# adobe-research/DiffusionHandles

Hardware: AMD Instinct MI355X
Metric: guided-denoise steps/sec at 512x512 (SD2-depth) (higher is better)
Workload: dtype f16; 1 GPU; single 512x512 edit per GPU, SD2-depth (865.9M params, seeded random weights), guided phase: 3 x (fwd + energy + bwd-to-latent) + CFG fwd (B=2) + DDIM step; resolution=512, edits_per_gpu=1, correspondences=24906, parallelism=independent edits, one process per GPU, no collectives

## Files before the change

diffusionhandles_amd/_lib.py:

```python
import ctypes
import os

import torch

_HERE = os.path.dirname(os.path.abspath(__file__))
LIB_PATH = os.environ.get("DIFFHANDLES_LIB") or os.path.join(_HERE, "libdiffhandles_hip.so")
_LIB = None

c_p = ctypes.c_void_p
c_i = ctypes.c_int
c_f = ctypes.c_float
c_d = ctypes.c_double
c_sz = ctypes.c_size_t


class UNetConfig(ctypes.Structure):
    _fields_ = [("in_channels", c_i), ("out_channels", c_i), ("n_levels", c_i),
                ("block_out_channels", c_i * 4), ("layers_per_block", c_i), ("heads", c_i * 4),
                ("cross_attention_dim", c_i), ("norm_groups", c_i), ("sample_size", c_i),
                ("text_len", c_i), ("max_batch", c_i), ("dtype", c_i), ("max_diff_batch", c_i)]


class VAEConfig(ctypes.Structure):
    _fields_ = [("latent_channels", c_i), ("out_channels", c_i), ("block_out_channels", c_i * 4),
# ... 70 lines not shown
    "dh_text_encoder_bytes": (c_sz, [c_p]),
    "dh_text_encoder_encode": (c_i, [c_p, c_p, c_i, c_i, c_p, c_p]),
    "dh_gemm_profile_begin": (c_i, []),
    "dh_gemm_profile_end": (c_i, [ctypes.POINTER(c_d), ctypes.POINTER(ctypes.c_int64), ctypes.POINTER(c_d)]),
    "dh_gemm_profile_bytes": (c_i, [ctypes.POINTER(c_d)]),
    "dh_ddim_cfg_step": (c_i, [c_p, c_p, c_p, c_p, c_f, c_f, c_f, c_i, c_p]),
    "dh_latent_update": (c_i, [c_p, c_p, c_p, c_f, c_f, c_i, c_p]),
    "dh_adam_step": (c_i, [c_p, c_p, c_p, c_p, c_f, c_f, c_f, c_f, c_i, c_i, c_p]),
    "dh_mse_fwd_bwd": (c_i, [c_p, c_p, c_i, c_p, c_p, c_p]),
    "dh_latent_update_strided": (c_i, [c_p, c_p, c_p, c_i, c_i, c_f, c_f, c_i, c_p]),
    "dh_pack_sample": (c_i, [c_p, c_p, c_i, c_i, c_p, c_i, c_i, c_i, c_i, c_p]),
    "dh_unet_io_ptr": (c_i, [c_p, c_i, c_i, ctypes.POINTER(c_p), ctypes.POINTER(c_sz)]),
    "dh_mse_cotangent": (c_i, [c_p, c_p, c_i, c_f, c_f, c_p, c_p, c_p, c_p]),
    "dh_adam_step_scaled": (c_i, [c_p, c_p, c_p, c_p, c_p, c_f, c_f, c_f, c_f, c_i, c_i, c_p]),
    "dh_mse_cotangent_batch": (c_i, [c_p, c_p, c_i, c_i, c_f, c_f, c_d, c_p, c_p, c_p, c_p, c_p, c_p]),
    "dh_adam_step_scaled_batch": (c_i, [c_p, c_p, c_p, c_p, c_p, c_p, c_f, c_f, c_f, c_f, c_i, c_i, c_i, c_p]),
    "dh_latent_update_guarded": (c_i, [c_p, c_p, c_p, c_i, c_i, c_f, c_i, c_i, c_p, c_i, c_i, c_p, c_p, c_i, c_i, c_p]),
    "dh_ddim_cfg_step_flagged": (c_i, [c_p, c_p, c_p, c_p, c_f, c_f, c_f, c_i, c_i, c_p, c_i, c_i, c_p]),
}

c_l = ctypes.c_long
DEBUG_SIGNATURES = {
    "dh_dbg_gemm": (c_i, [c_i, c_p, c_l, c_p, c_i, c_i, c_i, c_i, c_i, c_i, c_i, c_i, c_i, c_i, c_i, c_p, c_p, c_i, c_i,
                          c_p, c_l, c_p, c_l, c_i, c_p, c_sz, c_p]),
    "dh_dbg_gemm_groupnorm": (c_i, [c_i, c_p, c_l, c_p, c_i, c_i, c_i, c_i, c_i, c_i, c_i, c_p, c_p, c_p, c_sz, c_i, c_i, c_p, c_p, c_f, c_i,
                                    c_p, c_p, c_p, ctypes.POINTER(c_i), c_p]),
    "dh_dbg_gemm_groupnorm_bwd": (c_i, [c_i, c_p, c_l, c_p, c_i, c_i, c_i, c_i, c_i, c_i, c_i, c_p, c_p, c_sz, c_i, c_i, c_p, c_p, c_p, c_p, c_i,
                                        c_p, c_p, ctypes.POINTER(c_i), c_p]),
    "dh_dbg_gemm_groupnorm_res": (c_i, [c_i, c_p, c_l, c_p, c_i, c_i, c_i, c_i, c_i, c_i, c_i, c_p, c_p, c_l, c_p, c_p, c_sz, c_i, c_i, c_p, c_p,
                                    c_f, c_i, c_p, c_p, c_p, ctypes.POINTER(c_i), c_p]),
    "dh_dbg_gemm_groupnorm_bwd_res": (c_i, [c_i, c_p, c_l, c_p, c_i, c_i, c_i, c_i, c_i, c_i, c_i, c_p, c_l, c_p, c_p, c_sz, c_i, c_i, c_p, c_p, c_p,
                                        c_p, c_i, c_p, c_p, ctypes.POINTER(c_i), c_p]),
    "dh_dbg_concat_groupnorm": (c_i, [c_i, c_p, c_i, c_p, c_i, c_p, c_i, c_i, c_i, c_p, c_p, c_f, c_i, c_p, c_p, c_p, c_p]),
    "dh_dbg_gemm_last_tile": (c_i, [ctypes.POINTER(c_i)]),
    "dh_dbg_unet_concat_ops": (c_i, [ctypes.POINTER(UNetConfig), ctypes.POINTER(c_i), c_i, ctypes.POINTER(c_i)]),
    "dh_dbg_gemm_lnfold": (c_i, [c_i, c_p, c_l, c_p, c_i, c_i, c_i, c_p, c_p, c_p, c_f, c_p, c_l, c_p]),
    "dh_dbg_gemm_glu": (c_i, [c_i, c_i, c_p, c_l, c_p, c_i, c_i, c_i, c_p, c_p, c_p, c_p, c_p, c_p]),
    "dh_dbg_gemm_glub_split": (c_i, [c_i, c_p, c_l, c_p, c_i, c_i, c_i, c_i, c_p, c_l, c_i, c_p, c_p, ctypes.POINTER(c_i), c_p]),
    "dh_dbg_unet_ff_fold": (c_i, [c_p, c_i, ctypes.POINTER(c_i), ctypes.POINTER(c_i), c_p, c_p, c_p]),
    "dh_dbg_gemm_family": (c_i, [c_i]),
    "dh_dbg_gemm_stage": (c_i, [c_i]),
    "dh_dbg_gemm_pp_variant": (c_i, [c_i, c_p]),
    "dh_dbg_gemm_pp_ablate": (c_i, [c_i]),
    "dh_dbg_gemm_pp_persist": (c_i, [c_i]),
    "dh_dbg_gemm_pp_glu": (c_i, [c_i]),
    "dh_dbg_gemm_pp_plan": (c_i, [c_i, c_i, c_i, c_i, c_i, c_i, c_sz, ctypes.POINTER(c_i), ctypes.POINTER(c_i), ctypes.POINTER(c_i)]),
    "dh_dbg_touch_tiled": (c_i, [c_sz, c_p]),
    "dh_dbg_groupnorm": (c_i, [c_i, c_p, c_p, c_p, c_p, c_p, c_p, c_p, c_p, c_i, c_i, c_i, c_i, c_f, c_i, c_i, c_p]),
    "dh_dbg_layernorm": (c_i, [c_i, c_p, c_p, c_p, c_p, c_p, c_p, c_p, c_p, c_i, c_i, c_f, c_p]),
    "dh_dbg_geglu": (c_i, [c_i, c_p, c_p, c_p, c_p, c_i, c_i, c_p]),
    "dh_dbg_attention": (c_i, [c_i, c_p, c_l, c_p, c_p, c_l, c_p, c_l, c_p, c_p, c_p, c_p, c_p, c_p, c_i, c_i, c_i, c_i, c_p]),
    "dh_dbg_attention_bwd_pair": (c_i, [c_i, c_p, c_l, c_p, c_p, c_l, c_p, c_l, c_p, c_p, c_p, c_p, c_p, c_p, c_i, c_i, c_i, c_i, c_p, c_p]),
    "dh_dbg_pool2x2": (c_i, [c_i, c_p, c_p, c_i, c_i, c_i, c_i, c_i, c_p]),
    "dh_dbg_ellipse_offsets": (c_i, [c_i, ctypes.POINTER(ctypes.c_int32), c_i, ctypes.POINTER(c_i)]),
    "dh_dbg_lane_ops": (c_i, [c_p, c_p, c_p, c_p]),
}


def lib():
    global _LIB
    if _LIB is None:
        if not os.path.exists(LIB_PATH):
            raise RuntimeError(
                f"native HIP library not found at {LIB_PATH}; build it with "
                "`python -c 'import __graft_entry__ as g; g.build()'` (there is no CPU fallback)")
        handle = ctypes.CDLL(LIB_PATH)
        missing = []
# ... 40 lines not shown
```

diffusionhandles_amd/csrc/debug_api.cpp:

```cpp
#include <stdlib.h>

#include "unet_kernels.h"
using namespace dh;

static void* g_dbg_tiled = nullptr;

__global__ void k_dbg_touch(const uint4* p, size_t n16, unsigned* sink) {
  unsigned acc = 0;
  for (size_t i = (size_t)blockIdx.x * blockDim.x + threadIdx.x; i < n16; i += (size_t)gridDim.x * blockDim.x) { const uint4 v = p[i]; acc ^= v.x ^ v.y ^ v.z ^ v.w; }
  if (acc == 0x9e3779b9u && sink) sink[0] = acc;
}
extern "C" int dh_dbg_touch_tiled(size_t bytes, void* stream) {
  DH_REQUIRE(g_dbg_tiled != nullptr, "no tiled weights yet (call dh_dbg_gemm first)");
  hipLaunchKernelGGL(k_dbg_touch, dim3(512), dim3(256), 0, (hipStream_t)stream, (const uint4*)g_dbg_tiled, bytes / 16, (unsigned*)nullptr);
  DH_LAUNCH_CHECK();
  return DH_OK;
}

extern "C" int dh_dbg_gemm(int dtype, const void* A, long lda, const void* W, int M, int N, int K, int mode, int Hin,
                           int Win, int Cin, int Hout, int Wout, int stride, int up, const float* bias,
                           const float* rowvec, int rowvec_ld, int rows_per_batch, const void* R, long ldr, void* C,
                           long ldc, int act_silu, float* partial, size_t partial_elems, void* stream) {
  DH_REQUIRE(A && W && C && K % 64 == 0 && N % 64 == 0, "bad arguments (N, K must be multiples of 64)");
  void*& tiled = g_dbg_tiled;
// ... 20 lines not shown
}
extern "C" int dh_dbg_gemm_groupnorm_res(int dtype, const void* A, long lda, const void* W, int M, int N, int K, int mode, int Hin, int Win,
                                     int Cin, const float* bias, const void* R, long ldr, void* C, float* partial, size_t partial_elems, int HW, int G,
                                     const float* gamma, const float* beta, float eps, int silu, void* Y, float* stats, float* scratch,
                                     int* have_out, void* stream) {
  DH_REQUIRE(A && W && C && Y && stats && scratch && gamma && beta && K % 64 == 0 && N % 64 == 0 && HW > 0 && M % HW == 0, "bad arguments");
  static void* tiled = nullptr;
  static size_t cap = 0;
  const size_t need = (size_t)N * K * 2;
  if (need > cap) {
    if (tiled) (void)hipFree(tiled);
    DH_CHECK_HIP(hipMalloc(&tiled, need));
    cap = need;
  }
  launch_tile_weights(dtype, W, tiled, N, K, (hipStream_t)stream, mode != 0 ? Cin : 0);
  GemmArgs g;
  g.A = A; g.lda = lda; g.W = tiled; g.M = M; g.N = N; g.K = K; g.mode = mode; g.Hin = Hin; g.Win = Win; g.Cin = Cin;
  g.Hout = Hin; g.Wout = Win; g.stride = 1; g.up = 0; g.bias = bias; g.R = R; g.ldr = ldr; g.C = C; g.ldc = N;
  g.partial = partial; g.partial_elems = partial_elems;
  int have = 0;
  g.gn_part = scratch; g.gn_HW = HW; g.gn_G = G; g.gn_done = &have;
  launch_gemm(dtype, g, (hipStream_t)stream);
  launch_groupnorm_fwd(dtype, C, gamma, beta, Y, stats, scratch, M / HW, HW, N, G, eps, silu, (hipStream_t)stream, have);
  if (have_out) *have_out = have;
  DH_LAUNCH_CHECK();
  return DH_OK;
}
extern "C" int dh_dbg_gemm_groupnorm(int dtype, const void* A, long lda, const void* W, int M, int N, int K, int mode, int Hin, int Win,
                                     int Cin, const float* bias, void* C, float* partial, size_t partial_elems, int HW, int G,
                                     const float* gamma, const float* beta, float eps, int silu, void* Y, float* stats, float* scratch,
                                     int* have_out, void* stream) {
  return dh_dbg_gemm_groupnorm_res(dtype, A, lda, W, M, N, K, mode, Hin, Win, Cin, bias, nullptr, N, C, partial, partial_elems, HW, G,
                                   gamma, beta, eps, silu, Y, stats, scratch, have_out, stream);
}
extern "C" int dh_dbg_gemm_groupnorm_bwd_res(int dtype, const void* A, long lda, const void* W, int M, int N, int K, int mode, int Hin,
                                         int Win, int Cin, const void* R, long ldr, void* C, float* partial, size_t partial_elems, int HW, int G, const void* x,
                                         const float* gamma, const float* beta, const float* stats, int silu, void* dx,
                                         float* scratch, int* have_out, void* stream) {
  DH_REQUIRE(A && W && C && x && dx && stats && scratch && gamma && beta && K % 64 == 0 && N % 64 == 0 && HW > 0 && M % HW == 0, "bad arguments");
  static void* tiled = nullptr;
  static size_t cap = 0;
  const size_t need = (size_t)N * K * 2;
  if (need > cap) {
    if (tiled) (void)hipFree(tiled);
    DH_CHECK_HIP(hipMalloc(&tiled, need));
    cap = need;
  }
  launch_tile_weights(dtype, W, tiled, N, K, (hipStream_t)stream, mode != 0 ? Cin : 0);
  GemmArgs g;
  g.A = A; g.lda = lda; g.W = tiled; g.M = M; g.N = N; g.K = K; g.mode = mode; g.Hin = Hin; g.Win = Win; g.Cin = Cin;
  g.Hout = Hin; g.Wout = Win; g.stride = 1; g.up = 0; g.R = R; g.ldr = ldr; g.C = C; g.ldc = N;
  g.partial = partial; g.partial_elems = partial_elems;
  int have = 0;
  g.gnb_x = x; g.gnb_ldx = N; g.gnb_gamma = gamma; g.gnb_beta = beta; g.gnb_stats = stats; g.gnb_silu = silu;
  g.gn_part = scratch; g.gn_HW = HW; g.gn_G = G; g.gn_done = &have;
  launch_gemm(dtype, g, (hipStream_t)stream);
  launch_groupnorm_bwd(dtype, x, C, gamma, beta, stats, dx, scratch, M / HW, HW, N, G, silu, 0, (hipStream_t)stream, have, GnBwdSplit());
  if (have_out) *have_out = have;
  DH_LAUNCH_CHECK();
  return DH_OK;
}
extern "C" int dh_dbg_gemm_groupnorm_bwd(int dtype, const void* A, long lda, const void* W, int M, int N, int K, int mode, int Hin,
                                         int Win, int Cin, void* C, float* partial, size_t partial_elems, int HW, int G, const void* x,
                                         const float* gamma, const float* beta, const float* stats, int silu, void* dx,
                                         float* scratch, int* have_out, void* stream) {
  return dh_dbg_gemm_groupnorm_bwd_res(dtype, A, lda, W, M, N, K, mode, Hin, Win, Cin, nullptr, N, C, partial, partial_elems, HW, G, x,
// ... 151 lines not shown
```

diffusionhandles_amd/csrc/gemm.hip:

```cpp
#include <stdlib.h>

#include <vector>

#include <hip/hip_ext.h>

#include "gemm_k.h"

namespace dh {

struct GemmProf {
  bool on = false;
  std::vector<hipEvent_t> ev;
  size_t used = 0;
  double flops = 0;
  double bytes = 0;
  hipEvent_t e0 = nullptr, e1 = nullptr;
};
static GemmProf g_prof;
static int g_buf_stage = 1;
static int g_pp_force = 0;
struct GemmTileReport {
  int bm, bn, kg, stages, mw, splits, pp, gn_epi, reduce_gn;
};
static thread_local GemmTileReport g_last_tile;
// ... 43 lines not shown
}
template <class T>
__device__ __forceinline__ void epilogue_store(const GemmK& p, int m, int n, float v0, float v1, float v2, float v3,
                                               bool have_r = false, uint2 rpre = make_uint2(0, 0), bool have_b = false,
                                               float4 bpre = make_float4(0.f, 0.f, 0.f, 0.f)) {
  *reinterpret_cast<uint2*>(reinterpret_cast<T*>(p.C) + (size_t)m * p.ldc + n) =
      epilogue_pack<T>(p, m, n, v0, v1, v2, v3, have_r, rpre, have_b, bpre);
}

template <class T>
__device__ __forceinline__ float epilogue_scalar(const GemmK& p, int m, int n, float v) {
  if (p.bias) v += p.bias[n];
  if (p.rowvec) v += p.rowvec[(size_t)div_small(m, p.inv_rows_per_batch) * p.rowvec_ld + n];
  if (p.act_silu) v = v / (1.f + __expf(-v));
  if (p.R) v += to_f32<T>(reinterpret_cast<const T*>(p.R)[(size_t)m * p.ldr + n]);
  return to_f32<T>(from_f32<T>(v));
}

__device__ uint4 g_zero_page[8];

__device__ __forceinline__ void dma16(const void* gsrc, unsigned lds_dst) {
  unsigned keep;
  asm volatile("s_mov_b32 %0, m0\n\ts_mov_b32 m0, %2\n\ts_nop 0\n\tglobal_load_lds_dwordx4 %1, off\n\ts_mov_b32 m0, %0"
               : "=&s"(keep) : "v"(gsrc), "s"(lds_dst) : "memory");
}

__device__ __forceinline__ void dma16_nt(const void* gsrc, unsigned lds_dst) {
  unsigned keep;
  asm volatile("s_mov_b32 %0, m0\n\ts_mov_b32 m0, %2\n\ts_nop 0\n\tglobal_load_lds_dwordx4 %1, off nt\n\ts_mov_b32 m0, %0"
               : "=&s"(keep) : "v"(gsrc), "s"(lds_dst) : "memory");
}

typedef int buf_v4i __attribute__((ext_vector_type(4)));
__device__ __forceinline__ void buf_dma16(unsigned voff, buf_v4i rsrc, unsigned soff, unsigned lds_dst) {
  unsigned tmp;
  soff = __builtin_amdgcn_readfirstlane(soff);
  lds_dst = __builtin_amdgcn_readfirstlane(lds_dst);
  asm volatile("s_mov_b32 m0, %4\n\ts_mov_b32 %0, %3\n\tbuffer_load_dwordx4 %1, %2, %0 offen lds"
               : "=&s"(tmp) : "v"(voff), "s"(rsrc), "s"(soff), "s"(lds_dst) : "memory");
}
__device__ __forceinline__ unsigned buf_mask_oob(unsigned nt, unsigned sh, unsigned voff) {
  return ((nt << sh) & 0x80000000u) | voff;
}

template <int N> __device__ __forceinline__ void wait_vmcnt() { asm volatile("s_waitcnt vmcnt(%0)" ::"n"(N) : "memory"); }

enum { GM_DENSE = 0, GM_CONV_S1 = 1, GM_GENERIC = 2 };
#ifdef DH_TUNING
#define LNF_ABL(bit) && !(p.lnf_abl & (bit))
#define LEAN_ABL && !(p.lnf_abl & 8)
#define DH_STAMP(i) do { if (p.ts && blockIdx.x == 0 && blockIdx.y == 0 && blockIdx.z == 0 && threadIdx.x == 0) p.ts[i] = __builtin_amdgcn_s_memtime(); } while (0)
#define DH_STAMP_T(kt, j) do { if (p.ts && (kt) < 40 && blockIdx.x == 0 && blockIdx.y == 0 && blockIdx.z == 0 && threadIdx.x == 0) p.ts[8 + 3 * (kt) + (j)] = __builtin_amdgcn_s_memtime(); } while (0)
#else
#define DH_STAMP_T(kt, j) do { } while (0)
#define LNF_ABL(bit)
#define LEAN_ABL
#define DH_STAMP(i) do { } while (0)
#endif

typedef _Float16 v2h __attribute__((ext_vector_type(2)));
typedef __bf16 v2b __attribute__((ext_vector_type(2)));
typedef unsigned u4v __attribute__((ext_vector_type(4)));
template <class T> __device__ __forceinline__ void frag_sums(const uint4& f, float& s1, float& s2);
template <> __device__ __forceinline__ void frag_sums<f16>(const uint4& f_in, float& s1, float& s2) {
  const v2h one = {(_Float16)1.f, (_Float16)1.f};
  u4v f = __builtin_bit_cast(u4v, f_in);
  asm("" : "+v"(f));
  const unsigned w[4] = {f[0], f[1], f[2], f[3]};
#pragma unroll
  for (int i = 0; i < 4; ++i) {
    const v2h h = __builtin_bit_cast(v2h, w[i]);
    s1 = __builtin_amdgcn_fdot2(h, one, s1, false);
    s2 = __builtin_amdgcn_fdot2(h, h, s2, false);
// ... 68 lines not shown
    const int m = m0 + 8 * (wave + NWV * (j * WG + grp)) + prow;
    a_ok[j] = m < p.M;
    if (MODE == GM_DENSE) {
      a_off[j] = (long)(a_ok[j] ? m : p.M - 1) * p.lda + lchunk * 8;
      a_oy[j] = a_ox[j] = 0;
    } else {
      const int hw = p.Hout * p.Wout;
      const int b = div_small(m, inv_hw), r = m - b * hw;
      a_oy[j] = div_small(r, inv_w);
      a_ox[j] = r - a_oy[j] * p.Wout;
      if (MODE == GM_CONV_S1) a_off[j] = (((long)b * p.Hin + a_oy[j]) * p.Win + a_ox[j]) * p.lda + lchunk * 8;
      else a_off[j] = (long)b * p.Hin * p.Win;
    }
  }
  unsigned a_taps[NPA];
#pragma unroll
  for (int j = 0; j < NPA; ++j) {
    a_taps[j] = 0;
    if (MODE == GM_CONV_S1 && a_ok[j]) {
#pragma unroll
      for (int t = 0; t < 9; ++t)
        if ((unsigned)(a_oy[j] + t / 3 - 1) < (unsigned)p.Hin && (unsigned)(a_ox[j] + t % 3 - 1) < (unsigned)p.Win) a_taps[j] |= 1u << t;
    }
  }
  const T* Wg = reinterpret_cast<const T*>(p.W);
  const int KT = p.K >> 6;
  const T* b_ptr[NPB];
#pragma unroll
  for (int j = 0; j < NPB; ++j) {
    const int row = 8 * (wave + NWV * (j * WG + grp));
    b_ptr[j] = Wg + ((size_t)((n0 + row) >> 6) * KT) * 4096 + (size_t)((n0 + row) & 63) * 64 + lane * 8;
  }
  int tap = 0, c0 = 0;
  if (MODE != GM_DENSE) { const int kt0 = kbeg >> 6, ch = kt0 / 9; tap = kt0 - ch * 9; c0 = ch * BK; }
  typedef int bv4i __attribute__((ext_vector_type(4)));
  bv4i ra = {0, 0, 0, 0}, rw = {0, 0, 0, 0};
  unsigned bv_a[NPA], bv_nt[NPA], bs_w[NPB];
  unsigned bs_tap = 0, bs_sh = 0;
  unsigned bs_step_px = 0, bs_step_row = 0; int bs_kx = 0;
  const unsigned bv_w = lane * 16;
  if constexpr (BUF) {
    const unsigned a_bias = MODE == GM_CONV_S1 ? (unsigned)((p.Win + 1) * (int)p.lda * 2) : 0u;
    const size_t a_base = (size_t)p.A - a_bias;
    ra[0] = (int)(unsigned)a_base; ra[1] = (int)((a_base >> 32) & 0xffff); ra[2] = (int)(p.pp_a_bytes + a_bias); ra[3] = 0x00020000;
    rw[0] = (int)(unsigned)(size_t)p.W; rw[1] = (int)(((size_t)p.W >> 32) & 0xffff); rw[2] = (int)p.pp_w_bytes; rw[3] = 0x00020000;
#pragma unroll
    for (int j = 0; j < NPA; ++j) {
      const int m = m0 + 8 * (wave + NWV * (j * WG + grp)) + prow;
      if (MODE == GM_DENSE) {
        bv_a[j] = a_ok[j] ? (unsigned)m * (unsigned)((int)p.lda * 2) + (unsigned)lchunk * 16u : 0x80000000u;
        bv_nt[j] = 0;
      } else {
        const int hw = p.Hout * p.Wout;
        const int b = div_small(m, inv_hw);
        (void)hw;
        bv_a[j] = (unsigned)((b * p.Hin + a_oy[j]) * p.Win + a_ox[j]) * (unsigned)((int)p.lda * 2) + (unsigned)lchunk * 16u;
        bv_nt[j] = ~a_taps[j];
      }
    }
#pragma unroll
    for (int j = 0; j < NPB; ++j) {
      const int n = n0 + 8 * (wave_s + NWV * (j * WG + grp));
      bs_w[j] = (unsigned)(((n >> 6) * KT) * 8192 + (n & 63) * 128);
    }
    if (MODE == GM_CONV_S1) {
      const int ky = tap / 3, kx = tap - ky * 3;
      bs_tap = (unsigned)((ky * p.Win + kx) * (int)p.lda + c0) * 2u;
// ... 29 lines not shown
        const long toff = ((long)(ky - 1) * p.Win + (kx - 1)) * p.lda + c0;
        const bool ok = (a_taps[j] & (1u << tap)) != 0;
        const T* ptr = Ag + a_off[j] + toff;
        dma16(ok ? ptr : zero, sbase + (j * WG + grp) * (NWV * 1024));
      } else {
        const int ky = tap / 3, kx = tap - ky * 3;
        bool ok = a_ok[j];
        int sy, sx;
        if (p.mode == A_CONV3) {
          const int iy = a_oy[j] * p.stride + ky - p.pad, ix = a_ox[j] * p.stride + kx - p.pad;
          ok = ok && iy >= 0 && ix >= 0 && iy < (p.Hin << p.up) && ix < (p.Win << p.up);
          sy = iy >> p.up; sx = ix >> p.up;
        } else {
          const int ty = a_oy[j] + ky - 1, tx = a_ox[j] + kx - 1;
          ok = ok && ty >= 0 && tx >= 0 && !(ty & 1) && !(tx & 1) && (ty >> 1) < p.Hin && (tx >> 1) < p.Win;
          sy = ty >> 1; sx = tx >> 1;
        }
        sy = sy < 0 ? 0 : (sy >= p.Hin ? p.Hin - 1 : sy);
        sx = sx < 0 ? 0 : (sx >= p.Win ? p.Win - 1 : sx);
        const T* ptr = Ag + (a_off[j] + (long)sy * p.Win + sx) * p.lda + c0 + lchunk * 8;
        dma16(ok ? ptr : zero, sbase + (j * WG + grp) * (NWV * 1024));
      }
    } else {
      const int j = q - NPA;
#ifdef DH_TUNING
      if (p.w_nt) dma16_nt(b_ptr[j] + (size_t)(k0 >> 6) * 4096, sbase + BM * 128 + (j * WG + grp) * (NWV * 1024));
      else
#endif
      dma16(b_ptr[j] + (size_t)(k0 >> 6) * 4096, sbase + BM * 128 + (j * WG + grp) * (NWV * 1024));
    }
  };
  auto next_tile = [&]() {
    if constexpr (BUF && MODE == GM_CONV_S1) {
      ++tap; ++bs_kx;
      const bool row_end = bs_kx == 3;
      bs_tap += row_end ? bs_step_row : bs_step_px;
      bs_kx = row_end ? 0 : bs_kx;
      if (tap == 9) { tap = 0; c0 += BK; bs_tap = (unsigned)c0 * 2u; }
      bs_sh = 31u - (unsigned)tap;
      return;
    }
    if (MODE != GM_DENSE) { if (++tap == 9) { tap = 0; c0 += BK; } }
  };
  auto issue = [&](int kt, int stage) {
#pragma unroll
    for (int q = 0; q < NP; ++q) issue_piece(kt, stage, q);
    next_tile();
  };

  v16f acc[TM][TN];
#pragma unroll
  for (int i = 0; i < TM; ++i)
#pragma unroll
    for (int j = 0; j < TN; ++j)
#pragma unroll
      for (int r = 0; r < 16; ++r) acc[i][j][r] = 0.f;

  const int wn_u = __builtin_amdgcn_readfirstlane(wn);
  float ln1[TM], ln2[TM];
#pragma unroll
  for (int i = 0; i < TM; ++i) { ln1[i] = 0.f; ln2[i] = 0.f; }

#pragma unroll
  for (int s = 0; s < ST - 1; ++s)
    if (s < ntiles) issue(s, s);
  DH_STAMP(1);

  constexpr bool PRE = TM * TN <= 8;
  const bool pre_r = PRE && p.R != nullptr && p.pre_r && p.splits == 1 && (WG == 1 || grp == 0) && (KG == 1 || kg == 0) &&
                     (GLU != 2 || !glub_tile_is_glu(n0, p.glub_f));
  constexpr bool PRE_B = PRE && !(MW == 2 && BN == 320) && WNS == 2;
  const bool pre_b = PRE_B && p.bias != nullptr && p.pre_r && p.splits == 1;
  float4 bpre[PRE_B ? TN : 1][4];
  if (pre_b) {
#pragma unroll
// ... 491 lines not shown
#ifdef DH_TUNING
    if (p.ts) { asm volatile("s_waitcnt vmcnt(0)" ::: "memory"); DH_STAMP(7); }
#endif
    return;
  }

#pragma unroll
  for (int i = 0; i < TM; ++i) {
    const int m = m0 + wm * RPW + i * 32 + ln;
    if (m >= p.M) continue;
#pragma unroll
    for (int j = 0; j < TN; ++j)
#pragma unroll
      for (int g = 0; g < 4; ++g) {
        const int n = n0 + wn * CPW + j * 32 + 8 * g + 4 * hi;
        if (n >= p.N) continue;
        if (p.splits > 1) {
          float4 o = make_float4(acc[i][j][4 * g], acc[i][j][4 * g + 1], acc[i][j][4 * g + 2], acc[i][j][4 * g + 3]);
          *reinterpret_cast<float4*>(p.partial + ((size_t)blockIdx.z * p.M + m) * p.N + n) = o;
        } else {
          epilogue_store<T>(p, m, n, acc[i][j][4 * g], acc[i][j][4 * g + 1], acc[i][j][4 * g + 2], acc[i][j][4 * g + 3], pre_r,
                            rpre[i][j][g], pre_b, bpre[PRE_B ? j : 0][g]);
        }
      }
  }
}

template <class T>
__global__ void k_tile_weights(const T* src, T* dst, int N, int K, int conv_cin) {
  const size_t idx = (size_t)blockIdx.x * blockDim.x + threadIdx.x;
  if (idx >= (size_t)N * K) return;
  const int n = (int)(idx / K);
  int k = (int)(idx - (size_t)n * K);
  if (conv_cin) { const int tap = k / conv_cin; k = conv_k_index(tap, k - tap * conv_cin); }
  dst[wt_index(n, k, K)] = src[idx];
}
void launch_tile_weights(int dtype, const void* src, void* dst, int N, int K, hipStream_t st, int conv_cin) {
  const unsigned nb = (unsigned)(((size_t)N * K + 255) / 256);
  hipLaunchKernelGGL((k_tile_weights<unsigned short>), dim3(nb), dim3(256), 0, st, (const unsigned short*)src, (unsigned short*)dst, N, K, conv_cin);
}

template <class T>
__global__ void k_splitk_reduce(const GemmK p) {
  const size_t q = (size_t)blockIdx.x * blockDim.x + threadIdx.x;
  const size_t total = (size_t)p.M * p.N / 4;
  if (q >= total) return;
  const size_t e = q * 4;
  const int m = (int)((unsigned)e / (unsigned)p.N), n = (int)((unsigned)e - (unsigned)m * (unsigned)p.N);
  const bool have_r = p.R != nullptr, have_b = p.bias != nullptr;
  const uint2 rpre = have_r ? *reinterpret_cast<const uint2*>(reinterpret_cast<const T*>(p.R) + (size_t)m * p.ldr + n) : make_uint2(0, 0);
  const float4 bpre = have_b ? *reinterpret_cast<const float4*>(p.bias + n) : make_float4(0.f, 0.f, 0.f, 0.f);
  const size_t slab = (size_t)p.M * p.N;
  float4 s = make_float4(0.f, 0.f, 0.f, 0.f);
  int z = 0;
  for (; z + 4 <= p.splits; z += 4) {
    float4 v[4];
#pragma unroll
    for (int j = 0; j < 4; ++j) v[j] = *reinterpret_cast<const float4*>(p.partial + (size_t)(z + j) * slab + e);
#pragma unroll
    for (int j = 0; j < 4; ++j) { s.x += v[j].x; s.y += v[j].y; s.z += v[j].z; s.w += v[j].w; }
  }
  for (; z < p.splits; ++z) {
    const float4 v = *reinterpret_cast<const float4*>(p.partial + (size_t)z * slab + e);
    s.x += v.x; s.y += v.y; s.z += v.z; s.w += v.w;
  }
  epilogue_store<T>(p, m, n, s.x, s.y, s.z, s.w, have_r, rpre, have_b, bpre);
}
// ... 294 lines not shown
#else
  dim3 grid(tm, tn, splits);
#endif
  hipEvent_t e0 = nullptr, e1 = nullptr;
  if (g_prof.on) {
    if (g_prof.used + 2 > g_prof.ev.size()) {
      const size_t old = g_prof.ev.size();
      g_prof.ev.resize(old + 4096);
      for (size_t i = old; i < g_prof.ev.size(); ++i) (void)hipEventCreate(&g_prof.ev[i]);
    }
    e0 = g_prof.ev[g_prof.used++];
    e1 = g_prof.ev[g_prof.used++];
    g_prof.flops += 2.0 * (double)k.M * (double)k.N * (double)k.K;
    const double esz = 2.0;
    double a_elems = (double)k.M * k.K;
    if (k.mode != A_DENSE && k.Hout > 0 && k.Wout > 0) a_elems = (double)k.M / ((double)k.Hout * k.Wout) * k.Hin * k.Win * k.Cin;
    double c_elems = (double)k.M * k.N * (k.C ? 1.0 : 0.0) + (k.R ? (double)k.M * k.N : 0.0);
    if (k.glu_y) c_elems += 0.5 * (double)k.M * k.N;
    if (k.glub_x) c_elems += 4.0 * (double)k.M * k.glub_f - (k.C ? (double)k.M * k.glub_f : 0.0);
    if (k.gn_epi == 2) c_elems += (double)k.M * k.N;
    g_prof.bytes += esz * (a_elems + (double)k.N * k.K + c_elems);
    g_prof.e0 = e0; g_prof.e1 = e1;
  }
  int gm = GM_GENERIC;
  if (k.mode == A_DENSE) gm = GM_DENSE;
  else if (k.mode == A_CONV3 && k.stride == 1 && k.up == 0 && k.pad == 1) gm = GM_CONV_S1;
  if (!use_pp) {
    k.pp_a_bytes = 0; k.pp_w_bytes = 0;
    size_t ab = 0;
    if (k.mode == A_DENSE) ab = ((size_t)(k.M - 1) * k.lda + k.K) * 2;
    else if (k.Hout > 0 && k.Wout > 0 && k.M % (k.Hout * k.Wout) == 0)
      ab = (size_t)(k.M / (k.Hout * k.Wout)) * k.Hin * k.Win * (size_t)k.lda * 2;
    const size_t wb = (size_t)align_up((size_t)k.N, 64) * k.K * 2;
    const bool conv_ok = k.mode == A_DENSE || (k.Cin % 64 == 0 && k.K == 9 * k.Cin);
    if ((g_buf_stage & 1) && ab > 0 && conv_ok && ab + (size_t)(k.Win + 1) * k.lda * 2 < 0x7ff00000ull && wb < 0x7ff00000ull && k.lda % 8 == 0 &&
        ((size_t)k.A & 15) == 0 && ((size_t)k.W & 15) == 0) {
      k.pp_a_bytes = (unsigned)ab; k.pp_w_bytes = (unsigned)wb;
    }
  }
#ifdef DH_TUNING
  static const int kAbl = getenv("DH_GEMM_ABLATE") ? atoi(getenv("DH_GEMM_ABLATE")) : 0;
  if (kAbl == 1 && BM == 128 && BN == 128) { hipLaunchKernelGGL((k_gemm_dma<T, 128, 128, 4, GM_CONV_S1, 1>), grid, dim3(256), 0, st, k); }
  else if (kAbl == 2 && BM == 128 && BN == 128) { hipLaunchKernelGGL((k_gemm_dma<T, 128, 128, 4, GM_CONV_S1, 2>), grid, dim3(256), 0, st, k); }
  else if (kAbl == 3 && BM == 128 && BN == 128) { hipLaunchKernelGGL((k_gemm_dma<T, 128, 128, 4, GM_DENSE, 1>), grid, dim3(256), 0, st, k); }
  else if (kAbl == 1 && mw2 && gm == GM_CONV_S1) { hipLaunchKernelGGL((k_gemm_dma<T, 256, 128, 3, GM_CONV_S1, 1, 1, 1, 2>), grid, dim3(512), 0, st, k); }
  else if (kAbl == 2 && mw2 && gm == GM_CONV_S1) { hipLaunchKernelGGL((k_gemm_dma<T, 256, 128, 3, GM_CONV_S1, 2, 1, 1, 2>), grid, dim3(512), 0, st, k); }
  else if (kAbl == 1 && mw2 && gm == GM_DENSE && !lnf) { hipLaunchKernelGGL((k_gemm_dma<T, 256, 128, 3, GM_DENSE, 1, 1, 1, 2>), grid, dim3(512), 0, st, k); }
  else if (kAbl == 2 && mw2 && gm == GM_DENSE && !lnf) { hipLaunchKernelGGL((k_gemm_dma<T, 256, 128, 3, GM_DENSE, 2, 1, 1, 2>), grid, dim3(512), 0, st, k); }
  else if (force_tile == 1) launch_tile<T, 64, 64, 4, 1, 1, 1>(gm, lnf, grid, st, k);
  else if (force_tile == 2) launch_tile<T, 128, 64, 3, 1, 2, 1>(gm, lnf, grid, st, k);
  else if (force_tile == 3) launch_tile<T, 128, 64, 5, 1, 1, 1>(gm, lnf, grid, st, k);
  else if (force_tile == 4) launch_tile<T, 128, 128, 4, 1, 1, 2>(gm, lnf, grid, st, k);
  else if (force_tile == 5) launch_tile<T, 128, 128, 4, 1, 1, 1>(gm, lnf, grid, st, k);
  else if (force_tile == 6) launch_tile<T, 256, 128, 3, 1, 1, 2>(gm, lnf, grid, st, k);
  else if (force_tile == 7) launch_tile<T, 128, 160, 4, 1, 1, 1>(gm, false, grid, st, k);
  else
#endif
  if (use_pp) { pp.splits = splits; g_last_tile.bm = pp.bm; g_last_tile.bn = pp.bn; launch_gemm_pp(dtype, k, pp, st, g_prof.e0, g_prof.e1); }
  else if (t160) launch_tile<T, 128, 160, 4, 1, 1, 1>(gm, false, grid, st, k);
  else if (mw2) launch_tile<T, 256, 128, 3, 1, 1, 2>(gm, lnf, grid, st, k, glu);
  else if (BM == 128 && BN == 128 && (glu || (kMw128 && tiles_per_split >= kMw128))) launch_tile<T, 128, 128, 4, 1, 1, 2>(gm, lnf, grid, st, k, glu);
  else if (kTwoPerCu && BM == 128 && BN == 64 && tiles * splits > 256 && tiles * splits <= 512)
    launch_tile<T, 128, 64, 3, 1, 1, 1>(gm, lnf, grid, st, k);
  else if (BM == 128 && BN == 64 && tiles_per_split >= kKg2MinKt) launch_tile<T, 128, 64, 3, 1, 2, 1>(gm, lnf, grid, st, k);
  else if (BN == 320) launch_tile<T, 128, 320, 2, 1, 1, 2>(gm, false, grid, st, k);
  else if (BM == 64) launch_tile<T, 64, 64, 4, 1, 1, 1>(gm, lnf, grid, st, k, glu);
  else if (BN == 128 && kManyBlocks > 0 && tiles * splits >= kManyBlocks) launch_tile<T, 128, 128, 2, 1, 1, 1>(gm, lnf, grid, st, k);
  else if (BN == 128) launch_tile<T, 128, 128, 4, 1, 1, 1>(gm, lnf, grid, st, k);
  else launch_tile<T, 128, 64, 5, 1, 1, 1>(gm, lnf, grid, st, k);
  g_prof.e0 = g_prof.e1 = nullptr;
  g_last_tile.splits = splits; g_last_tile.pp = use_pp ? 1 : 0; g_last_tile.gn_epi = k.gn_epi;
  if (k.gn_epi) *gn_done = k.gn_S;
  if (splits > 1) {
    if (k.gn_part && k.gn_G > 0 && k.gn_HW > 0 && k.N % k.gn_G == 0 && (GN_GB * (k.N / k.gn_G)) % 8 == 0 &&
        GN_GB * (k.N / k.gn_G) <= 2048 && k.M % k.gn_HW == 0) {
      k.gn_S = gn_slices(k.gn_HW, k.M / k.gn_HW);
      if (k.gnb_x) hipLaunchKernelGGL((k_splitk_reduce_gn<T, true>), dim3(k.gn_S, cdiv(k.gn_G, GN_GB), k.M / k.gn_HW), dim3(256), 0, st, k);
      else hipLaunchKernelGGL((k_splitk_reduce_gn<T, false>), dim3(k.gn_S, cdiv(k.gn_G, GN_GB), k.M / k.gn_HW), dim3(256), 0, st, k);
      g_last_tile.reduce_gn = 1;
      if (gn_done) *gn_done = 1;
    } else if (k.lnb_x && lnb_done && !k.bias && !k.rowvec && !k.R && !k.act_silu && k.N % 8 == 0 && k.ldc == k.N) {
      launch_splitk_reduce_ln_bwd(dtype, k.partial, splits, k.lnb_x, k.lnb_gamma, k.lnb_stats, k.lnb_add, k.lnb_dx, k.M, k.N, st, k.lnb_ldx);
      *lnb_done = 1;
    } else {
      const size_t groups = (size_t)k.M * k.N / 4;
      hipLaunchKernelGGL((k_splitk_reduce<T>), dim3((unsigned)((groups + 255) / 256)), dim3(256), 0, st, k);
    }
  }
}
#undef DH_KNOB

double launch_gemm(int dtype, const GemmArgs& a, hipStream_t st) {
  GemmK k;
  k.A = a.A; k.lda = a.lda; k.W = a.W; k.M = a.M; k.N = a.N; k.K = a.K;
  k.mode = a.mode; k.Hin = a.Hin; k.Win = a.Win; k.Cin = a.Cin; k.Hout = a.Hout; k.Wout = a.Wout;
  k.stride = a.stride; k.up = a.up; k.pad = a.pad;
  k.bias = a.bias; k.rowvec = a.rowvec; k.rowvec_ld = a.rowvec_ld;
  k.rows_per_batch = a.rows_per_batch > 0 ? a.rows_per_batch : 1;
  k.inv_rows_per_batch = 1.f / (float)k.rows_per_batch;
  k.R = a.R; k.ldr = a.ldr; k.C = a.C; k.ldc = a.ldc; k.act_silu = a.act_silu;
  k.partial = a.partial; k.splits = 1; k.k_per_split = a.K;
  k.pre_r = 1;
  k.wide_store = a.N % 32 == 0 && a.ldc % 8 == 0 && ((size_t)a.C & 15) == 0;
  k.ln_s = a.ln_s; k.ln_t = a.ln_t; k.ln_stats = a.ln_stats; k.ln_eps = a.ln_eps;
  k.gn_part = a.gn_part; k.gn_HW = a.gn_HW; k.gn_G = a.gn_G; k.gn_S = 0;
  k.gnb_x = a.gnb_x; k.gnb_ldx = a.gnb_ldx; k.gnb_gamma = a.gnb_gamma; k.gnb_beta = a.gnb_beta; k.gnb_stats = a.gnb_stats;
  k.gnb_silu = a.gnb_silu;
  k.lnb_x = a.lnb_x; k.lnb_ldx = a.lnb_ldx > 0 ? a.lnb_ldx : a.N;
  k.lnb_gamma = a.lnb_gamma; k.lnb_stats = a.lnb_stats; k.lnb_add = a.lnb_add; k.lnb_dx = a.lnb_dx;
  k.glu_y = a.glu_y; k.glu_ldy = a.glu_ldy; k.glub_x = a.glub_x; k.glub_dx = a.glub_dx;
  k.glub_f = a.glub_x && a.glub_f > 0 && a.glub_f < a.N ? a.glub_f : a.N;
  if (k.glub_f < a.N) {
    if (k.C) k.C = reinterpret_cast<unsigned short*>(k.C) - k.glub_f;
    if (k.R) k.R = reinterpret_cast<const unsigned short*>(k.R) - k.glub_f;
  } else if (a.glub_x) {
    k.C = nullptr;
  }
  if (a.gn_done) *a.gn_done = 0;
  if (a.lnb_done) *a.lnb_done = 0;
  if (dtype == DH_DTYPE_F16) gemm_dispatch<f16>(k, a.partial_elems, st, a.gn_done, a.lnb_done, dtype);
  else gemm_dispatch<bf16>(k, a.partial_elems, st, a.gn_done, a.lnb_done, dtype);
  return 2.0 * (double)a.M * (double)a.N * (double)a.K;
}

}

#ifdef DH_TUNING
extern "C" int dh_dbg_gemm_timeline(unsigned long long* ts) { dh::g_gemm_ts = ts; return DH_OK; }
#endif

extern "C" int dh_dbg_gemm_family(int force) {
  DH_REQUIRE(force >= 0 && force <= 2, "family: 0 policy, 1 k_gemm_dma, 2 k_gemm_pp");
  dh::g_pp_force = force;
  return DH_OK;
}

extern "C" int dh_dbg_gemm_stage(int buf) {
  dh::g_buf_stage = buf;
  return DH_OK;
}

extern "C" int dh_dbg_gemm_last_tile(int* out) {
  DH_REQUIRE(out != nullptr, "null pointer");
  const dh::GemmTileReport& r = dh::g_last_tile;
  const int v[9] = {r.bm, r.bn, r.kg, r.stages, r.mw, r.splits, r.pp, r.gn_epi, r.reduce_gn};
  for (int i = 0; i < 9; ++i) out[i] = v[i];
  return DH_OK;
}

extern "C" int dh_gemm_profile_begin(void) {
  dh::g_prof.on = true;
  dh::g_prof.used = 0;
  dh::g_prof.flops = 0;
  dh::g_prof.bytes = 0;
  return DH_OK;
}
extern "C" int dh_gemm_profile_bytes(double* bytes) {
  if (bytes) *bytes = dh::g_prof.bytes;
  return DH_OK;
}
extern "C" int dh_gemm_profile_end(double* ms_total, int64_t* launches, double* flops) {
  using namespace dh;
  g_prof.on = false;
  double ms = 0;
  if (g_prof.used >= 2) DH_CHECK_HIP(hipEventSynchronize(g_prof.ev[g_prof.used - 1]));
  for (size_t i = 0; i + 1 < g_prof.used; i += 2) {
    float t = 0;
    DH_CHECK_HIP(hipEventElapsedTime(&t, g_prof.ev[i], g_prof.ev[i + 1]));
    ms += t;
  }
  if (ms_total) *ms_total = ms;
  if (launches) *launches = (int64_t)(g_prof.used / 2);
  if (flops) *flops = g_prof.flops;
  return DH_OK;
}
```

diffusionhandles_amd/csrc/gemm_k.h:

```cpp
#pragma once
#include "unet_kernels.h"

namespace dh {

typedef _Float16 v8h __attribute__((ext_vector_type(8)));
typedef __bf16 v8b __attribute__((ext_vector_type(8)));
typedef float v16f __attribute__((ext_vector_type(16)));

template <class T> struct Mfma;
template <> struct Mfma<f16> {
  static __device__ __forceinline__ v16f run(uint4 a, uint4 b, v16f c) {
    return __builtin_amdgcn_mfma_f32_32x32x16_f16(__builtin_bit_cast(v8h, a), __builtin_bit_cast(v8h, b), c, 0, 0, 0);
  }
};
template <> struct Mfma<bf16> {
  static __device__ __forceinline__ v16f run(uint4 a, uint4 b, v16f c) {
    return __builtin_amdgcn_mfma_f32_32x32x16_bf16(__builtin_bit_cast(v8b, a), __builtin_bit_cast(v8b, b), c, 0, 0, 0);
  }
};

struct GemmK {
  const void* A; long lda;
  const void* W;
  int M, N, K;
  int mode, Hin, Win, Cin, Hout, Wout, stride, up, pad;
  const float* bias;
  const float* rowvec; int rowvec_ld; int rows_per_batch; float inv_rows_per_batch;
  const void* R; long ldr;
  void* C; long ldc;
  int act_silu;
  int pre_r;
  int wide_store;
#ifdef DH_TUNING
  int w_nt;
  unsigned long long* ts;
  int lnf_abl;
#endif
  const float* ln_s; const float* ln_t; float* ln_stats; float ln_eps;
  float* partial;
  int splits, k_per_split;
  float* gn_part; int gn_HW, gn_G, gn_S;
  int gn_epi, gn_cpg;
  const void* gnb_x; long gnb_ldx; const float *gnb_gamma, *gnb_beta, *gnb_stats; int gnb_silu;
  const void* lnb_x; long lnb_ldx; const float *lnb_gamma, *lnb_stats; const void* lnb_add; void* lnb_dx;
  void* glu_y; long glu_ldy; const void* glub_x; void* glub_dx;
  int glub_f;
  int pp_tm, pp_tn, pp_order, pp_nwork; unsigned pp_a_bytes, pp_w_bytes;
  unsigned long long* pp_ts;
};


__host__ __device__ constexpr bool glub_tile_is_glu(int n0, int glub_f) { return n0 < glub_f; }
__host__ __device__ constexpr bool glub_split_ok(int BN, int glub_f) { return BN > 0 && glub_f % BN == 0; }

struct PpPlan { int bm = 0, bn = 0, splits = 1; };
bool gemm_pp_plan(const GemmK& k, size_t partial_elems, int force, PpPlan* plan);
void launch_gemm_pp(int dtype, const GemmK& k, const PpPlan& plan, hipStream_t st, hipEvent_t e0, hipEvent_t e1);

}
```

diffusionhandles_amd/csrc/gemm_pp.hip:

```cpp
#include <hip/hip_ext.h>

#include <type_traits>
#include <utility>

#include "gemm_k.h"

namespace dh {

typedef float v4f __attribute__((ext_vector_type(4)));
typedef int v4i __attribute__((ext_vector_type(4)));
typedef unsigned lane_u2p __attribute__((ext_vector_type(2)));

template <class T> struct Mfma16;
template <> struct Mfma16<f16> {
  typedef v8h frag;
  static __device__ __forceinline__ v4f run(frag a, frag b, v4f c) { return __builtin_amdgcn_mfma_f32_16x16x32_f16(a, b, c, 0, 0, 0); }
};
template <> struct Mfma16<bf16> {
  typedef v8b frag;
  static __device__ __forceinline__ v4f run(frag a, frag b, v4f c) { return __builtin_amdgcn_mfma_f32_16x16x32_bf16(a, b, c, 0, 0, 0); }
};

constexpr unsigned PP_OOB = 0x80000000u;

// ... 94 lines not shown
    const int m = m0 + 8 * (qa0 + j) + prow;
    const int lchunk = (lane & 7) ^ ((4 * ((qa0 + j) & 1) + (prow >> 1)) & 7);
    a_ok[j] = m < p.M;
    a_taps[j] = 0; a_oy[j] = 0; a_ox[j] = 0; a_lch[j] = 0;
    if (MODE == PP_DENSE) {
      a_voff[j] = (a_ok[j] ? (unsigned)m * (unsigned)(p.lda * 2) + lchunk * 16 : PP_OOB) - 1024u * j;
    } else {
      const int hw = p.Hout * p.Wout;
      const int b = m / hw, r = m - b * hw;
      a_oy[j] = r / p.Wout;
      a_ox[j] = r - a_oy[j] * p.Wout;
      if (MODE == PP_CONV_S1) {
        a_voff[j] = (unsigned)((b * p.Hin + a_oy[j]) * p.Win + a_ox[j]) * (unsigned)(p.lda * 2) + lchunk * 16 - 1024u * j;
        if (a_ok[j]) {
#pragma unroll
          for (int t = 0; t < 9; ++t)
            if ((unsigned)(a_oy[j] + t / 3 - 1) < (unsigned)p.Hin && (unsigned)(a_ox[j] + t % 3 - 1) < (unsigned)p.Win) a_taps[j] |= 1u << t;
        }
      } else {
        a_voff[j] = (unsigned)(b * p.Hin * p.Win);
        a_lch[j] = lchunk * 16 + a_bias - 1024u * j;
      }
    }
  }
  const unsigned w_voff = lane * 16;
  const int KT = p.K >> 6;
  unsigned w_soff[NPB0];
#pragma unroll
  for (int j = 0; j < NPB0; ++j) {
    const int n = n0 + 8 * (qb0 + j);
    w_soff[j] = (unsigned)(((n >> 6) * KT) * 8192 + (n & 63) * 128) + (unsigned)(kbeg >> 6) * 8192u - 1024u * j;
  }
  int tap = 0, c0 = 0;
  if (MODE != PP_DENSE) { const int kt0 = kbeg >> 6, ch = kt0 / 9; tap = kt0 - ch * 9; c0 = ch * 64; }
  int kt_issue = 0;
  int kti = 0;
  int issued = 0;

  const unsigned lds0 = (unsigned)(size_t)((__attribute__((address_space(3))) unsigned char*)smem);
  const unsigned m0_a = __builtin_amdgcn_readfirstlane(lds0 + qa0 * 1024), m0_w = __builtin_amdgcn_readfirstlane(lds0 + BM * 128 + qb0 * 1024);
  auto issue_piece = [&](int stage, auto Qc, bool first) {
    constexpr int Q = decltype(Qc)::value;
    if constexpr (Q < NPA) {
      constexpr int j = Q;
      if (j == 0 || first) pp_set_m0(m0_a + stage * STAGE);
      if (MODE == PP_DENSE) {
        pp_dma<j * 1024>(a_voff[j], ra, (unsigned)(kbeg + kti * 64) * 2u);
      } else if (MODE == PP_CONV_S1) {
        const int ky = tap / 3, kx = tap - ky * 3;
        const unsigned soff = (unsigned)((ky * p.Win + kx) * (int)p.lda + c0) * 2u;
        const bool ok = (a_taps[j] >> tap) & 1u;
        pp_dma<j * 1024>(ok ? a_voff[j] : PP_OOB - 1024u * j, ra, soff);
      } else {
        const int ky = tap / 3, kx = tap - ky * 3;
        bool ok = a_ok[j];
        int sy, sx;
        if (p.mode == A_CONV3) {
          const int iy = a_oy[j] * p.stride + ky - p.pad, ix = a_ox[j] * p.stride + kx - p.pad;
          ok = ok && iy >= 0 && ix >= 0 && iy < (p.Hin << p.up) && ix < (p.Win << p.up);
          sy = iy >> p.up; sx = ix >> p.up;
        } else {
          const int ty = a_oy[j] + ky - 1, tx = a_ox[j] + kx - 1;
          ok = ok && ty >= 0 && tx >= 0 && !(ty & 1) && !(tx & 1) && (ty >> 1) < p.Hin && (tx >> 1) < p.Win;
          sy = ty >> 1; sx = tx >> 1;
        }
        const unsigned off = (a_voff[j] + (unsigned)(sy * p.Win + sx)) * (unsigned)(p.lda * 2) + a_lch[j];
        pp_dma<j * 1024>(ok ? off : PP_OOB - 1024u * j, ra, (unsigned)c0 * 2u);
      }
      ++issued;
    } else {
      constexpr int j = Q - NPA;
      if (j < NPB1 || g == 0) {
        if (j == 0 || first) pp_set_m0(m0_w + stage * STAGE);
        pp_dma<j * 1024>(w_voff, rw, w_soff[j] + (unsigned)kti * 8192u);
        ++issued;
      }
    }
  };
  auto issue_range = [&](int stage, auto LOc, auto HIc) {
    constexpr int LO = decltype(LOc)::value, HI = decltype(HIc)::value;
    if constexpr (LO < HI) {
      [&]<int... I>(std::integer_sequence<int, I...>) {
        (issue_piece(stage, std::integral_constant<int, LO + I>{}, I == 0), ...);
      }(std::make_integer_sequence<int, HI - LO>{});
    }
  };
  auto next_tile = [&]() {
    ++kt_issue;
    kti = __builtin_amdgcn_readfirstlane(kt_issue);
    if (MODE != PP_DENSE) { if (++tap == 9) { tap = 0; c0 += 64; } }
  };
  int rpre_n = 0;
  auto wait_tile = [&](int u) {
    int n = issued - (u + 1) * npw;
    if (n < 0) n = 0;
    if (u < NST - 1) n += rpre_n;
    pp_wait_vm_dyn<0, 31>(n);
  };

  v4f acc[TM][TN];
#pragma unroll
  for (int i = 0; i < TM; ++i)
#pragma unroll
    for (int j = 0; j < TN; ++j) acc[i][j] = (v4f){0.f, 0.f, 0.f, 0.f};

  stamp();
#pragma unroll
  for (int s = 0; s < NST - 1; ++s) {
    if (s < nt) {
      issue_range(s, std::integral_constant<int, 0>{}, std::integral_constant<int, NP0>{});
      next_tile();
    }
  }
  constexpr int NRP = TN / 2, NR1 = TN & 1;
  const int nb = n0 + g * CPW;
  const bool has_r = p.R != nullptr && p.splits == 1;
  const bool pre_r = has_r && !(VAR & PPV_NO_RPRE);
  uint4 rp16[TM][NRP > 0 ? NRP : 1];
  uint2 rp8[TM];
  if (pre_r) {
#pragma unroll
    for (int i = 0; i < TM; ++i) {
      const int m = m0 + wm * RPW + 16 * i + l15;
// ... 310 lines not shown
static size_t pp_a_bytes(const GemmK& k) {
  if (k.mode == A_DENSE) return ((size_t)(k.M - 1) * k.lda + k.K) * 2;
  const size_t B = (size_t)k.M / ((size_t)k.Hout * k.Wout);
  return B * k.Hin * k.Win * (size_t)k.lda * 2;
}

static int pp_device_cus() {
  static int cus = 0;
  if (cus == 0) {
    int dev = 0, n = 0;
    if (hipGetDevice(&dev) == hipSuccess && hipDeviceGetAttribute(&n, hipDeviceAttributeMultiprocessorCount, dev) == hipSuccess && n >= 8) cus = n - n % 8;
    else { (void)hipGetLastError(); cus = 256; }
  }
  return cus;
}

static int g_pp_glu = -1;
bool gemm_pp_plan(const GemmK& k, size_t partial_elems, int force, PpPlan* plan) {
  if (force == 1) return false;
  if (k.ln_s || k.act_silu) return false;
  const int glu = k.glu_y ? 1 : (k.glub_x ? 2 : 0);
  const bool glu_here = force == 2 || g_pp_glu > 0 || (g_pp_glu < 0 && ((glu == 1 && k.M >= 2048) || k.M >= 32768));
  if (glu && !glu_here) return false;
  if (glu == 2 && k.glub_f > 0 && k.glub_f < k.N) return false;
  if (glu && (k.mode != A_DENSE || k.N % 128 || k.rowvec || k.R || (glu == 1 && (k.glu_ldy % 8 || ((size_t)k.glu_y & 15))) ||
              (glu == 2 && (((size_t)k.glub_x & 15) || ((size_t)k.glub_dx & 15))))) return false;
  if (k.rowvec && (k.rowvec_ld % 4 || ((size_t)k.rowvec & 15))) return false;
  if (k.K % 64 || k.M <= 0 || (!k.C && !glu)) return false;
  if (k.N % 160 && k.N % 128) return false;
  if (k.N % 64) return false;
  if (k.bias && ((size_t)k.bias & 15)) return false;
  if ((k.C && (k.ldc % 8 || ((size_t)k.C & 15))) || k.lda % 8 || ((size_t)k.A & 15) || ((size_t)k.W & 15)) return false;
  if (k.R && (k.ldr % 8 || ((size_t)k.R & 15))) return false;
  if (k.mode != A_DENSE && (k.Hout <= 0 || k.Wout <= 0 || k.M % (k.Hout * k.Wout) || k.Cin % 64 || k.K != 9 * k.Cin)) return false;
  const size_t ab = pp_a_bytes(k) + (size_t)(k.Win + 1) * k.lda * 2, wb = (size_t)k.N * k.K * 2;
  if (ab >= 0x7ff00000ull || wb >= 0x7ff00000ull) return false;
  const int ktiles = k.K / 64;
  const int bn = (k.N % 160 == 0 && !glu) ? 160 : 128;
  const int tn = k.N / bn;
  const long t256 = (long)cdiv(k.M, 256) * tn, t128 = (long)cdiv(k.M, 128) * tn;
  int bm = 0, splits = 1;
  const int cus = pp_device_cus(), fill = cus - cus / 8;
  if (t256 >= fill) bm = 256;
  else if (t128 >= fill) bm = 128;
  else if (!glu && k.partial && ktiles >= 64 && t256 >= 64 && k.M >= 1024 && k.M <= 4096) {
    bm = 256;
    splits = (int)(cus / t256);
    if (splits > ktiles / 8) splits = ktiles / 8;
    if (splits > 8) splits = 8;
    const size_t fit = partial_elems / ((size_t)k.M * k.N);
    if ((size_t)splits > fit) splits = (int)fit;
    if (splits < 2) bm = 0;
  }
  if (force == 2 && bm == 0) { bm = k.M > 128 ? 256 : 128; splits = 1; }
  if (bm == 0) return false;
  plan->bm = bm; plan->bn = bn; plan->splits = splits;
  return true;
}

constexpr int PP_SHIP_256 = PPV_K64 | (1 << PPV_NDIM_SHIFT), PP_SHIP_128 = PPV_K64 | (3 << PPV_NDIM_SHIFT);
static int g_pp_persist = 1;
static int g_pp_ablate = 0;
static int g_pp_variant = -1;
static unsigned long long* g_pp_ts = nullptr;

template <class T, int BM, int BN, int NST, int VAR>
static void pp_launch_tile(int mode, dim3 grid, hipStream_t st, const GemmK& k, hipEvent_t e0, hipEvent_t e1) {
// ... 46 lines not shown

void launch_gemm_pp(int dtype, const GemmK& kin, const PpPlan& plan, hipStream_t st, hipEvent_t e0, hipEvent_t e1) {
  GemmK k = kin;
  const int ktiles = k.K / 64;
  const int tiles_per_split = cdiv(ktiles, plan.splits);
  k.splits = cdiv(ktiles, tiles_per_split);
  k.k_per_split = tiles_per_split * 64;
  k.pp_tm = cdiv(k.M, plan.bm);
  k.pp_tn = k.N / plan.bn;
  k.pp_a_bytes = (unsigned)pp_a_bytes(k);
  k.pp_w_bytes = (unsigned)((size_t)k.N * k.K * 2);
  k.pp_ts = g_pp_ts;
  const double a_tot = (double)k.pp_a_bytes, w_tot = (double)k.pp_w_bytes;
  const double col_fastest = a_tot + 8.0 * w_tot;
  const double row_fastest = w_tot + (double)(k.pp_tn * k.splits < 8 ? k.pp_tn * k.splits : 8) * a_tot;
  k.pp_order = (row_fastest < col_fastest ? 1 : 0) | g_pp_ablate;
  k.pp_nwork = k.pp_tm * k.pp_tn * k.splits;
  int slots = pp_device_cus();
  if (g_pp_persist == 0 || k.pp_nwork <= slots) slots = k.pp_nwork;
  dim3 grid((unsigned)slots);
  const int mode = pp_mode(k);
  if (dtype == DH_DTYPE_F16) pp_launch<f16>(k, plan, mode, grid, st, e0, e1);
  else pp_launch<bf16>(k, plan, mode, grid, st, e0, e1);
}

}

extern "C" int dh_dbg_gemm_pp_plan(int M, int N, int K, int conv, int hw, int glu, size_t partial_elems, int* bm, int* bn, int* splits) {
  DH_REQUIRE(bm && bn && splits, "null pointer");
  static __attribute__((aligned(16))) unsigned char dummy[16];
  dh::GemmK k{};
  k.A = dummy; k.W = dummy; k.C = dummy; k.M = M; k.N = N; k.K = K; k.lda = conv ? K / 9 : K; k.ldc = N;
  k.mode = conv ? dh::A_CONV3 : dh::A_DENSE;
  if (conv) { k.Hin = k.Win = k.Hout = k.Wout = hw; k.Cin = K / 9; k.stride = 1; k.up = 0; k.pad = 1; }
  k.partial = partial_elems ? reinterpret_cast<float*>(dummy) : nullptr;
  if (glu == 1) { k.glu_y = dummy; k.glu_ldy = N / 2; }
  if (glu == 2) { k.glub_x = dummy; k.glub_dx = dummy; k.C = nullptr; }
  dh::PpPlan plan;
  const bool use = dh::gemm_pp_plan(k, partial_elems, 0, &plan);
  *bm = use ? plan.bm : 0; *bn = use ? plan.bn : 0; *splits = use ? plan.splits : 0;
  return DH_OK;
}
extern "C" int dh_dbg_gemm_pp_glu(int on) {
  dh::g_pp_glu = on;
  return DH_OK;
}
extern "C" int dh_dbg_gemm_pp_persist(int on) {
  dh::g_pp_persist = on;
  return DH_OK;
}
extern "C" int dh_dbg_gemm_pp_ablate(int bits) {
#ifndef DH_PP_VARIANTS
  DH_REQUIRE(bits == 0, "timing ablations exist in the measurement build only (tools/lab.sh build-pp-variants)");
#endif
  dh::g_pp_ablate = bits & 0x300;
  return DH_OK;
}
extern "C" int dh_dbg_gemm_pp_variant(int variant, unsigned long long* ts) {
#ifndef DH_PP_VARIANTS
  DH_REQUIRE(variant < 0, "this build carries the shipped k_gemm_pp variants only (tools/lab.sh build-pp-variants)");
#endif
  DH_REQUIRE(variant >= -1 && variant < 256, "variant: bit 0 stamps, bit 1 all DMA inside the MFMA segment, bit 2 64-deep segments, bits 4-6 pieces inside the MFMA segment");
  dh::g_pp_variant = variant;
  dh::g_pp_ts = ts;
  return DH_OK;
}
```

diffusionhandles_amd/csrc/unet_engine.cpp:

```cpp
#include <stdlib.h>

#include <algorithm>
#include <map>
#include <numeric>
#include <vector>

#include "unet_kernels.h"

namespace dh {

enum OpType { OP_CONV_IN, OP_CONV_OUT, OP_GEMM, OP_GN, OP_LN, OP_ATTN, OP_GEGLU, OP_CONCAT, OP_TIMESTEP, OP_T2F };
enum ParamKind { PK_F32, PK_MAT };

struct Ten {
  size_t off = 0, goff = 0;
  size_t off_fo = 0;
  int rows = 0, C = 0;
  int ld = 0;
  int view = -1, col = 0;
  bool req_grad = true;
  bool persistent = false;
};

struct Wt {
  size_t fwd_off = 0, bwd_off = 0;
  int N = 0, K = 0, taps = 1;
  bool has_bwd = true, f32 = false;
  int glu_F = 0;
};

struct ParamInfo {
  std::string name;
  int ndim = 0;
  int64_t shape[4] = {0, 0, 0, 0};
  int kind = PK_F32;
  size_t f32_off = 0;
  int wt = -1;
  int row_off = 0;
  int glu_F = 0;
};

struct Op {
  int type = OP_GEMM;
  int in0 = -1, in1 = -1, out = -1, res = -1;
  int wt = -1;
  long bias_off = -1;
  long gamma_off = -1, beta_off = -1;
  int mode = A_DENSE, Hin = 0, Win = 0, Cin = 0, Hout = 0, Wout = 0, stride = 1, up = 0;
  int in_col = 0, in_cols = 0;
  long rowvec_off = -1; int rowvec_ld = 0;
  int act_silu = 0;
  float eps = 1e-5f; int silu = 0; int groups = 32; size_t stats_off = 0;
  int heads = 0, Nq = 0, Nk = 0, cross = 0, kv_col = 0; size_t lse_off = 0;
  int gn_next = -1;
  int ln_fold = -1, folded = 0;
  long ln_s_off = -1, ln_t_off = -1;
  int glu_op = -1, glub_op = -1;
};

struct FfFold {
  int wt_po = -1, wt_ffo = -1, wt = -1;
  long b_po = -1, b_ffo = -1, bias = -1;
};

}

using namespace dh;

struct dh_unet {
  dh_unet_config cfg;
  int dtype = DH_DTYPE_F16;
  std::vector<Ten> tens;
  std::vector<Wt> wts;
  std::vector<ParamInfo> params;
  std::vector<Op> ops;
  std::vector<FfFold> ffolds;
  std::map<std::string, int> pindex;
  size_t w16_elems = 0, pf_elems = 0, act_elems = 0, grad_elems = 0, f32_elems = 0;
  size_t fo_elems = 0;
  size_t partial_elems = 0, scratch_elems = 0, small_elems = 0;
  unsigned short *w16 = nullptr, *act = nullptr, *grad = nullptr, *scratch = nullptr;
  float *pf = nullptr, *f32a = nullptr, *partial = nullptr, *small = nullptr;
  int t_text = -1, t_kv = -1, t_conv_in_out = -1, t_final = -1, act_ids[3] = {-1, -1, -1};
  int act_op_end[3] = {0, 0, 0};
  int first_cross_op = 0;
  int saved_ops = 0;
  int temb_ops = 0, temb_rows = 0;
  float temb_t = 0.f;
  hipStream_t temb_stream = nullptr;
  uint64_t text_key = 0, kv_key = 0;
  int kv_rows = 0;
  hipStream_t kv_stream = nullptr;
  long temb_f32_off = -1;
  int temb_total = 0, kv_total = 0;
  float *in_sample = nullptr, *in_text = nullptr, *io_eps = nullptr, *out_dsample = nullptr, *out_dtext = nullptr, *t_dev = nullptr;
  std::map<uint64_t, hipGraphExec_t> graphs;
  std::map<uint64_t, double> graph_flops;
  bool use_graphs = true;
  long ones_off = -1, zeros_off = -1;
  bool fold_dirty = true;
  bool owns_weights = true;
  int n_shared = 0;
  int saved_batch = 0;
  const float* saved_sample = nullptr;
  std::vector<char> gready;
  double flops_fwd = 0, flops_bwd = 0;
  int64_t launches = 0;

  bool fo_mode = false;
// ... 54 lines not shown
    if (taps == 9) { p.ndim = 4; p.shape[0] = rows; p.shape[1] = cin; p.shape[2] = 3; p.shape[3] = 3; }
    else { p.ndim = 2; p.shape[0] = rows; p.shape[1] = cin; }
    u.pindex[name] = (int)u.params.size();
    u.params.push_back(p);
  }
  void bind_conv1x1(const std::string& name, int wt, int rows, int cin) {
    bind_mat(name, wt, rows, 0, cin, 1);
    ParamInfo& p = u.params.back();
    p.ndim = 4; p.shape[2] = 1; p.shape[3] = 1;
  }

  int gn(int x, const std::string& pre, float eps, bool silu) {
    const Ten tx = u.tens[x];
    Op o;
    o.type = OP_GN; o.in0 = x; o.out = tensor(tx.rows, tx.C);
    o.gamma_off = param_f32(pre + ".weight", tx.C);
    o.beta_off = param_f32(pre + ".bias", tx.C);
    o.eps = eps; o.silu = silu; o.groups = u.cfg.norm_groups;
    o.stats_off = f32_slot((size_t)maxB * o.groups * 2);
    u.ops.push_back(o);
    return o.out;
  }
  int ln(int x, const std::string& pre) {
    const Ten tx = u.tens[x];
    Op o;
    o.type = OP_LN; o.in0 = x; o.out = tensor(tx.rows, tx.C);
    o.gamma_off = param_f32(pre + ".weight", tx.C);
    o.beta_off = param_f32(pre + ".bias", tx.C);
    o.eps = 1e-5f;
    o.stats_off = f32_slot((size_t)maxB * tx.rows * 2);
    u.ops.push_back(o);
    return o.out;
  }
  int conv3(int x, const std::string& pre, int Cout, int Hs, int stride, int up, long temb_off, int res) {
    const Ten& tx = u.tens[x];
    const int Cin = tx.C;
    const int Hv = Hs << up, Ho = stride == 2 ? Hv / 2 : Hv;
    Op o;
    o.type = OP_GEMM; o.mode = A_CONV3; o.in0 = x; o.res = res;
    o.Hin = Hs; o.Win = Hs; o.Cin = Cin; o.Hout = Ho; o.Wout = Ho; o.stride = stride; o.up = up;
    o.wt = weight(Cout, 9 * Cin, 9);
    bind_mat(pre + ".weight", o.wt, Cout, 0, Cin, 9);
    o.bias_off = param_f32(pre + ".bias", Cout);
    if (temb_off >= 0) { o.rowvec_off = u.temb_f32_off + temb_off; o.rowvec_ld = u.temb_total; }
    o.out = tensor(Ho * Ho, Cout);
    u.ops.push_back(o);
    return o.out;
  }
  int linear_w(int x, int wt, long bias_off, int res, int in_col = 0, int in_cols = 0, bool silu = false,
               bool req_grad = true) {
    const Ten tx = u.tens[x];
    Op o;
    o.type = OP_GEMM; o.mode = A_DENSE; o.in0 = x; o.res = res; o.wt = wt; o.bias_off = bias_off;
    o.in_col = in_col; o.in_cols = in_cols ? in_cols : tx.C; o.act_silu = silu;
    o.out = tensor(tx.rows, u.wts[wt].N, req_grad);
    u.ops.push_back(o);
    return o.out;
  }
  int linear(int x, const std::string& pre, int N, bool bias, int res, bool as_conv1x1 = false) {
    const int K = u.tens[x].C;
    const int wt = weight(N, K);
    if (as_conv1x1) bind_conv1x1(pre + ".weight", wt, N, K); else bind_mat(pre + ".weight", wt, N, 0, K, 1);
    const long b = bias ? param_f32(pre + ".bias", N) : -1;
    return linear_w(x, wt, b, res);
  }
  int concat(int a, int b) {
    Op o;
    o.type = OP_CONCAT; o.in0 = a; o.in1 = b;
    o.out = tensor(u.tens[a].rows, u.tens[a].C + u.tens[b].C);
    u.ops.push_back(o);
    return o.out;
  }

  void fold_ln_into_last_gemm() {
    const int gi = (int)u.ops.size() - 1, li = gi - 1;
    Op& g = u.ops[gi];
    Op& l = u.ops[li];
    if (g.type != OP_GEMM || l.type != OP_LN || g.in0 != l.out || g.mode != A_DENSE || g.in_col != 0) return;
    const int N = u.wts[g.wt].N;
    g.ln_fold = li; l.folded = 1;
    g.ln_s_off = (long)u.pf_elems; u.pf_elems += align_up((size_t)N, 64);
    g.ln_t_off = (long)u.pf_elems; u.pf_elems += align_up((size_t)N, 64);
  }

  int temb_cursor = 0, kv_cursor = 0;
  int wt_temb = -1, wt_kv = -1;
  size_t temb_bias_off = 0;

  int resnet(int x, const std::string& pre, int Cout, int H) {
    const int Cin = u.tens[x].C;
    int h = gn(x, pre + ".norm1", 1e-5f, true);
    bind_mat(pre + ".time_emb_proj.weight", wt_temb, Cout, temb_cursor, u.cfg.block_out_channels[0] * 4, 1);
    param_f32_at(pre + ".time_emb_proj.bias", Cout, temb_bias_off + temb_cursor);
    const long toff = temb_cursor;
    temb_cursor += Cout;
    h = conv3(h, pre + ".conv1", Cout, H, 1, 0, toff, -1);
    h = gn(h, pre + ".norm2", 1e-5f, true);
    int sc = x;
    if (Cin != Cout) sc = linear(x, pre + ".conv_shortcut", Cout, true, -1, true);
    return conv3(h, pre + ".conv2", Cout, H, 1, 0, -1, sc);
  }

  int transformer(int x, const std::string& pre, int heads, int H) {
    const int C = u.tens[x].C, N = H * H;
    int h = gn(x, pre + ".norm", 1e-6f, false);
    int t0 = linear(h, pre + ".proj_in", C, true, -1);
    const std::string b = pre + ".transformer_blocks.0";
    int n1 = ln(t0, b + ".norm1");
    const int wqkv = weight(3 * C, C);
    bind_mat(b + ".attn1.to_q.weight", wqkv, C, 0, C, 1);
    bind_mat(b + ".attn1.to_k.weight", wqkv, C, C, C, 1);
    bind_mat(b + ".attn1.to_v.weight", wqkv, C, 2 * C, C, 1);
    int qkv = linear_w(n1, wqkv, -1, -1);
    fold_ln_into_last_gemm();
    Op a;
    a.type = OP_ATTN; a.in0 = qkv; a.heads = heads; a.Nq = N; a.Nk = N; a.cross = 0;
    a.out = tensor(N, C);
    a.lse_off = f32_slot((size_t)maxB * heads * N);
    u.ops.push_back(a);
    int t1 = linear(a.out, b + ".attn1.to_out.0", C, true, t0);
    int n2 = ln(t1, b + ".norm2");
    int q2 = linear(n2, b + ".attn2.to_q", C, false, -1);
    fold_ln_into_last_gemm();
    bind_mat(b + ".attn2.to_k.weight", wt_kv, C, kv_cursor, u.cfg.cross_attention_dim, 1);
    bind_mat(b + ".attn2.to_v.weight", wt_kv, C, kv_cursor + C, u.cfg.cross_attention_dim, 1);
    Op c;
    c.type = OP_ATTN; c.in0 = q2; c.in1 = u.t_kv; c.heads = heads; c.Nq = N; c.Nk = u.cfg.text_len; c.cross = 1;
    c.kv_col = kv_cursor;
    kv_cursor += 2 * C;
    c.out = tensor(N, C);
    c.lse_off = f32_slot((size_t)maxB * heads * N);
    u.ops.push_back(c);
    const int tg = tensor(N, 5 * C, false);
// ... 144 lines not shown
  for (size_t i = 0; i + 1 < u.ops.size(); ++i) {
    Op& o = u.ops[i];
    const Op& nx = u.ops[i + 1];
    if (nx.type == OP_GN && nx.in0 == o.out && (o.type == OP_GEMM || o.type == OP_CONCAT)) o.gn_next = (int)(i + 1);
  }
  { int cmax = 0;
    for (const Op& o : u.ops) if (o.type == OP_LN) cmax = std::max(cmax, u.tens[o.in0].C);
    u.ones_off = (long)u.pf_elems; u.pf_elems += align_up((size_t)cmax, 64);
    u.zeros_off = (long)u.pf_elems; u.pf_elems += align_up((size_t)cmax, 64); }
  layout_tensors(u);
  size_t biggest = 0;
  for (const Ten& t : u.tens) biggest = std::max(biggest, (size_t)t.rows * t.C * c.max_diff_batch);
  u.scratch_elems = biggest * 4 + 1024;
  for (const FfFold& f : u.ffolds) u.scratch_elems = std::max(u.scratch_elems, ff_fold_scratch(u.wts[f.wt_po].N));
  u.partial_elems = std::max<size_t>((size_t)48 << 20, biggest * 2);
  u.small_elems = (size_t)c.max_batch * 64 * 4096 + (size_t)c.max_batch * c.norm_groups * 4 + 4096;
  return DH_OK;
}


static void layout_tensors(dh_unet& u) {
  const size_t maxB = (size_t)u.cfg.max_batch, maxBd = (size_t)u.cfg.max_diff_batch;
  const int nt = (int)u.tens.size(), nops = (int)u.ops.size();
  u.tens[u.t_text].persistent = true;
  u.tens[u.t_kv].persistent = true;
  for (int i = 0; i < 3; ++i)
    if (u.act_ids[i] >= 0) u.tens[u.act_ids[i]].persistent = true;
  auto root = [&](int t) { return t >= 0 && u.tens[t].view >= 0 ? u.tens[t].view : t; };
  std::vector<int> first(nt, nops), last(nt, -1);
  auto rd = [&](int t, int oi) { t = root(t); if (t >= 0) { last[t] = std::max(last[t], oi); first[t] = std::min(first[t], oi); } };
  auto wr = [&](int t, int oi) { t = root(t); if (t >= 0) { first[t] = std::min(first[t], oi); last[t] = std::max(last[t], oi); } };
  for (int oi = 0; oi < nops; ++oi) {
    const Op& o = u.ops[oi];
    rd(o.in0, oi); rd(o.in1, oi); rd(o.res, oi); wr(o.out, oi);
    if (o.ln_fold >= 0) rd(u.ops[o.ln_fold].in0, oi);
    if (o.glu_op >= 0) wr(u.ops[o.glu_op].out, oi);
  }
  std::vector<char> written(nt, 0);
  for (const Op& o : u.ops) { if (o.out >= 0) written[root(o.out)] = 1; if (o.glu_op >= 0) written[root(u.ops[o.glu_op].out)] = 1; }
  for (int t = 0; t < nt; ++t)
    if (u.tens[t].view < 0 && (!written[t] || t == u.t_final)) {
      first[t] = 0; last[t] = nops; u.tens[t].persistent = u.tens[t].persistent || !written[t];
    }
  u.act_elems = 0; u.grad_elems = 0;
  for (Ten& t : u.tens) {
    if (t.view < 0) {
      t.off = u.act_elems;
      u.act_elems += align_up((size_t)t.rows * t.C * (t.persistent ? maxB : maxBd), 128);
    }
    if (t.req_grad) { t.goff = u.grad_elems; u.grad_elems += align_up((size_t)t.rows * t.C * maxBd, 128); }
  }
  struct Live { size_t off, end; int last; };
  std::vector<Live> live;
  for (const Ten& t : u.tens)
    if (t.persistent) live.push_back({t.off, t.off + align_up((size_t)t.rows * t.C * maxB, 128), nops + 1});
  std::vector<int> order(nt);
  std::iota(order.begin(), order.end(), 0);
  std::stable_sort(order.begin(), order.end(), [&](int a, int b) { return first[a] < first[b]; });
  size_t fo_end = 0;
  for (const Live& l : live) fo_end = std::max(fo_end, l.end);
  for (int t : order) {
    Ten& tt = u.tens[t];
    if (tt.view >= 0) continue;
    if (tt.persistent) { tt.off_fo = tt.off; continue; }
    if (last[t] < 0) { tt.off_fo = 0; continue; }
    const size_t size = align_up((size_t)tt.rows * tt.C * maxB, 128);
    live.erase(std::remove_if(live.begin(), live.end(), [&](const Live& l) { return l.last < first[t]; }), live.end());
// ... 8 lines not shown
    fo_end = std::max(fo_end, pos + size);
  }
  u.fo_elems = fo_end;
  u.act_elems = std::max(u.act_elems, fo_end);
  for (Ten& t : u.tens)
    if (t.view >= 0) {
      const Ten& r = u.tens[t.view];
      t.off = r.off + t.col; t.off_fo = r.off_fo + t.col; t.persistent = r.persistent;
    }
}

template <class D, bool TILED>
__global__ void k_load_weight(const float* src, int N, int C, int taps, D* fwd, long fwd_K, long row_off, D* bwd,
                              long bwd_K, long col_off, int Nb, float scale = 1.f, int glu_F = 0) {
  const size_t idx = (size_t)blockIdx.x * blockDim.x + threadIdx.x;
  if (idx >= (size_t)N * C * taps) return;
  const int tap = (int)(idx % taps);
  const int cc = (int)((idx / taps) % C);
  int nn = (int)(idx / ((size_t)taps * C));
  if (glu_F) nn = glu_col(nn >= glu_F ? nn - glu_F : nn, nn >= glu_F ? 1 : 0);
  const D v = from_f32<D>(src[idx] * scale);
  int fk = tap * C + cc, bk = (taps - 1 - tap) * Nb + (int)col_off + nn;
  if (TILED && taps == 9) { fk = conv_k_index(tap, cc); bk = conv_k_index(taps - 1 - tap, (int)col_off + nn); }
  const int fr = (int)row_off + nn;
  if (TILED) {
    fwd[wt_index(fr, fk, (int)fwd_K)] = v;
    if (bwd) bwd[wt_index(cc, bk, (int)bwd_K)] = v;
  } else {
    fwd[(size_t)fr * fwd_K + fk] = v;
    if (bwd) bwd[(size_t)cc * bwd_K + bk] = v;
  }
}

}
namespace dh {
void launch_load_weight(int dtype, const float* src, int N, int C, int taps, void* fwd, long fwd_K, long row_off, void* bwd,
                        long bwd_K, long col_off, int Nb, float scale, hipStream_t st) {
  const size_t total = (size_t)N * C * taps;
  const unsigned nb = (unsigned)((total + 255) / 256);
  if (dtype == DH_DTYPE_F32)
    hipLaunchKernelGGL((k_load_weight<float, false>), dim3(nb), dim3(256), 0, st, src, N, C, taps, (float*)fwd, fwd_K, row_off, (float*)bwd, bwd_K, col_off, Nb, scale);
  else if (dtype == DH_DTYPE_F16)
    hipLaunchKernelGGL((k_load_weight<f16, true>), dim3(nb), dim3(256), 0, st, src, N, C, taps, (f16*)fwd, fwd_K, row_off, (f16*)bwd, bwd_K, col_off, Nb, scale);
  else
    hipLaunchKernelGGL((k_load_weight<bf16, true>), dim3(nb), dim3(256), 0, st, src, N, C, taps, (bf16*)fwd, fwd_K, row_off, (bf16*)bwd, bwd_K, col_off, Nb, scale);
}
}
namespace {

template <class D>
__global__ void __launch_bounds__(256) k_fold_ln(const D* bwd, int bwd_K, const float* gamma, const float* beta, const float* bias,
                                                 D* fwd, int K, float* s_out, float* t_out) {
  __shared__ float sm[8];
  const int n = blockIdx.x;
  float s = 0.f, t = 0.f;
  for (int k = threadIdx.x; k < K; k += blockDim.x) {
    const float w = to_f32<D>(bwd[wt_index(k, n, bwd_K)]);
    const D wf = from_f32<D>(w * gamma[k]);
    fwd[wt_index(n, k, K)] = wf;
    s += to_f32<D>(wf);
    t += beta[k] * w;
  }
  s = block_sum(s, sm);
  __syncthreads();
  t = block_sum(t, sm);
  if (threadIdx.x == 0) { s_out[n] = s; t_out[n] = t + (bias ? bias[n] : 0.f); }
// ... 61 lines not shown
    g.A = po_plain; g.lda = C;
    g.W = u->w16 + ffo.bwd_off;
    g.mode = A_DENSE; g.M = C; g.N = 4 * C; g.K = C;
    g.C = prod; g.ldc = 4 * C;
    launch_gemm(u->dtype, g, st);
    hipLaunchKernelGGL((k_pack_ff_fold<D>), dim3(cdiv(5 * C * C, 256)), dim3(256), 0, st, (const D*)prod, (const D*)po_plain, C,
                       (D*)(u->w16 + wf.fwd_off), (D*)(u->w16 + wf.bwd_off));
    hipLaunchKernelGGL((k_fold_ff_bias<D>), dim3(C), dim3(256), 0, st, (const D*)po_plain, C, u->pf + f.b_ffo, u->pf + f.b_po,
                       u->pf + f.bias);
  }
}

static void fold_layernorms(dh_unet* u, hipStream_t st) {
  { int cmax = 0;
    for (const Op& o : u->ops) if (o.type == OP_LN) cmax = std::max(cmax, u->tens[o.in0].C);
    if (cmax > 0) {
      hipLaunchKernelGGL(k_fill_f32, dim3(cdiv(cmax, 256)), dim3(256), 0, st, u->pf + u->ones_off, cmax, 1.f);
      hipLaunchKernelGGL(k_fill_f32, dim3(cdiv(cmax, 256)), dim3(256), 0, st, u->pf + u->zeros_off, cmax, 0.f);
    } }
  for (const Op& g : u->ops) {
    if (g.type != OP_GEMM || g.ln_fold < 0) continue;
    const Op& l = u->ops[g.ln_fold];
    const Wt& w = u->wts[g.wt];
    const float* bias = g.bias_off >= 0 ? u->pf + g.bias_off : nullptr;
    if (u->dtype == DH_DTYPE_F16)
      hipLaunchKernelGGL((k_fold_ln<f16>), dim3(w.N), dim3(256), 0, st, (const f16*)(u->w16 + w.bwd_off), w.N, u->pf + l.gamma_off,
                         u->pf + l.beta_off, bias, (f16*)(u->w16 + w.fwd_off), w.K, u->pf + g.ln_s_off, u->pf + g.ln_t_off);
    else
      hipLaunchKernelGGL((k_fold_ln<bf16>), dim3(w.N), dim3(256), 0, st, (const bf16*)(u->w16 + w.bwd_off), w.N, u->pf + l.gamma_off,
                         u->pf + l.beta_off, bias, (bf16*)(u->w16 + w.fwd_off), w.K, u->pf + g.ln_s_off, u->pf + g.ln_t_off);
  }
  if (u->dtype == DH_DTYPE_F16) fold_ff_t<f16>(u, st);
  else fold_ff_t<bf16>(u, st);
  u->fold_dirty = false;
}

}

static int create_engine(const dh_unet_config* cfg, dh_unet* parent, dh_unet** out);
extern "C" int dh_unet_create(const dh_unet_config* cfg, dh_unet** out) {
  DH_REQUIRE(cfg && out, "null pointer");
  DH_REQUIRE(cfg->n_levels == 4, "n_levels must be 4");
  DH_REQUIRE(cfg->dtype == DH_DTYPE_F16 || cfg->dtype == DH_DTYPE_BF16, "dtype must be f16 or bf16");
  DH_REQUIRE(cfg->max_batch >= 1 && cfg->max_batch < 4096 && cfg->sample_size % 8 == 0 && cfg->sample_size >= 8, "bad batch / sample size");
  DH_REQUIRE((long)cfg->max_batch * cfg->sample_size * cfg->sample_size < (1L << 21), "max_batch * sample_size^2 must stay below 2^21 rows");
  DH_REQUIRE(cfg->norm_groups >= 1 && cfg->norm_groups <= 32, "1..32 GroupNorm groups");
  DH_REQUIRE(cfg->in_channels <= 8 && cfg->out_channels <= 8, "in/out channels must be <= 8");
  DH_REQUIRE(cfg->block_out_channels[0] <= 2048, "block_out_channels[0] must be <= 2048 (few-channel convolutions)");
  DH_REQUIRE(cfg->cross_attention_dim % 64 == 0, "cross_attention_dim must be a multiple of 64");
  for (int i = 0; i < 4; ++i) {
    DH_REQUIRE(cfg->block_out_channels[i] % 64 == 0, "block_out_channels must be multiples of 64");
    DH_REQUIRE(cfg->block_out_channels[i] == cfg->heads[i] * 64, "head dim must be 64");
    DH_REQUIRE(cfg->block_out_channels[i] % cfg->norm_groups == 0, "channels must divide into norm groups");
  }
  return create_engine(cfg, nullptr, out);
}

static int create_engine(const dh_unet_config* cfg, dh_unet* parent, dh_unet** out) {
  dh_unet* u = new dh_unet();
  u->cfg = *cfg;
  if (u->cfg.max_diff_batch <= 0 || u->cfg.max_diff_batch > u->cfg.max_batch) u->cfg.max_diff_batch = u->cfg.max_batch;
  u->dtype = cfg->dtype;
  int rc = build(*u);
  if (rc != DH_OK) { delete u; return rc; }
  auto fail = [&](hipError_t e, const char* what) {
    set_error(std::string(what) + ": " + hipGetErrorString(e));
// ... 90 lines not shown
  hipStream_t st = (hipStream_t)stream;
  const ParamInfo& p = u->params[i];
  if (p.kind == PK_F32) {
    if (p.glu_F) {
      hipLaunchKernelGGL(k_load_glu_bias, dim3(cdiv((int)p.shape[0], 256)), dim3(256), 0, st, src, u->pf + p.f32_off, p.glu_F);
      DH_LAUNCH_CHECK();
      return DH_OK;
    }
    DH_CHECK_HIP(hipMemcpyAsync(u->pf + p.f32_off, src, (size_t)p.shape[0] * 4, hipMemcpyDeviceToDevice, st));
    return DH_OK;
  }
  const Wt& w = u->wts[p.wt];
  const int N = (int)p.shape[0], C = (int)p.shape[1], taps = w.taps;
  const size_t total = (size_t)N * C * taps;
  const unsigned nb = (unsigned)((total + 255) / 256);
  const long fwd_ld = w.K;
  const long bwd_ld = (long)taps * w.N;
  if (w.f32) {
    float* f = u->pf + w.fwd_off;
    float* b = w.has_bwd ? u->pf + w.bwd_off : nullptr;
    hipLaunchKernelGGL((k_load_weight<float, false>), dim3(nb), dim3(256), 0, st, src, N, C, taps, f, fwd_ld, (long)p.row_off,
                       b, bwd_ld, (long)p.row_off, w.N);
  } else if (u->dtype == DH_DTYPE_F16) {
    f16* f = (f16*)(u->w16 + w.fwd_off);
    f16* b = w.has_bwd ? (f16*)(u->w16 + w.bwd_off) : nullptr;
    hipLaunchKernelGGL((k_load_weight<f16, true>), dim3(nb), dim3(256), 0, st, src, N, C, taps, f, fwd_ld, (long)p.row_off, b,
                       bwd_ld, (long)p.row_off, w.N, 1.f, w.glu_F);
  } else {
    bf16* f = (bf16*)(u->w16 + w.fwd_off);
    bf16* b = w.has_bwd ? (bf16*)(u->w16 + w.bwd_off) : nullptr;
    hipLaunchKernelGGL((k_load_weight<bf16, true>), dim3(nb), dim3(256), 0, st, src, N, C, taps, f, fwd_ld, (long)p.row_off, b,
                       bwd_ld, (long)p.row_off, w.N, 1.f, w.glu_F);
  }
  DH_LAUNCH_CHECK();
  return DH_OK;
}

extern "C" size_t dh_unet_weight_bytes(const dh_unet* u) { return u && u->owns_weights ? u->w16_elems * 2 + u->pf_elems * 4 : 0; }
extern "C" size_t dh_unet_workspace_bytes(const dh_unet* u) {
  return u ? (u->act_elems + u->grad_elems + u->scratch_elems) * 2 + (u->f32_elems + u->partial_elems + u->small_elems) * 4 : 0;
}

static void fill_gemm(dh_unet* u, const Op& o, int B, GemmArgs& g) {
  const Wt& w = u->wts[o.wt];
  const Ten& ti = u->tens[o.in0];
  const Ten& to = u->tens[o.out];
  g.A = u->aptr(o.in0) + o.in_col; g.lda = ti.ld;
  g.W = u->w16 + w.fwd_off;
  g.M = B * to.rows; g.N = w.N; g.K = w.K;
  g.mode = o.mode; g.Hin = o.Hin; g.Win = o.Win; g.Cin = o.Cin; g.Hout = o.Hout; g.Wout = o.Wout;
  g.stride = o.stride; g.up = o.up;
  g.bias = o.bias_off >= 0 ? u->pf + o.bias_off : nullptr;
  if (o.rowvec_off >= 0) { g.rowvec = u->f32a + o.rowvec_off; g.rowvec_ld = o.rowvec_ld; g.rows_per_batch = to.rows; }
  if (o.res >= 0) { g.R = u->aptr(o.res); g.ldr = u->tens[o.res].ld; }
  g.C = u->aptr(o.out); g.ldc = to.ld;
  g.act_silu = o.act_silu;
  g.partial = u->partial; g.partial_elems = u->partial_elems;
  if (o.ln_fold >= 0) {
    const Op& l = u->ops[o.ln_fold];
    if (use_ln_fold(u, B)) {
      g.A = u->aptr(l.in0); g.lda = u->tens[l.in0].ld;
      g.bias = nullptr;
      g.ln_s = u->pf + o.ln_s_off; g.ln_t = u->pf + o.ln_t_off; g.ln_stats = u->f32a + l.stats_off; g.ln_eps = l.eps;
    } else {
      g.bias = u->pf + o.ln_t_off;
    }
  }
}

static void forward_ops(dh_unet* u, int B, int n_ops, int first_op, bool kv_hit, bool save, hipStream_t st) {
  const int dt = u->dtype;
  const dh_unet_config& c = u->cfg;
  u->flops_fwd = 0;
  int gn_have = 0;
  if (!kv_hit) launch_f32_to_t(dt, u->in_text, u->aptr(u->t_text), (size_t)B * c.text_len * c.cross_attention_dim, st);
  for (int oi = first_op; oi < n_ops; ++oi) {
    const Op& o = u->ops[oi];
    if (kv_hit && oi == u->temb_ops) continue;
    switch (o.type) {
      case OP_TIMESTEP:
        launch_timestep_embedding(dt, u->t_dev, c.block_out_channels[0], B, u->aptr(o.out), st);
        break;
      case OP_T2F:
        launch_t_to_f32(dt, u->aptr(o.in0), u->f32a + u->temb_f32_off, (size_t)B * u->temb_total, 0, st);
        break;
      case OP_CONV_IN: {
        const Wt& w = u->wts[o.wt];
        launch_conv_small_fwd(dt, u->in_sample, 1, u->pf + w.fwd_off, u->pf + o.bias_off, u->aptr(o.out), 0, B, o.Hin, o.Hin,
                              o.Cin, w.N, st);
        u->flops_fwd += 2.0 * B * o.Hin * o.Hin * w.N * w.K;
        break;
      }
      case OP_CONV_OUT: {
        const Wt& w = u->wts[o.wt];
        launch_conv_small_fwd(dt, u->aptr(o.in0), 0, u->pf + w.fwd_off, u->pf + o.bias_off, u->io_eps, 1, B, o.Hin, o.Hin,
                              o.Cin, w.N, st);
        u->flops_fwd += 2.0 * B * o.Hin * o.Hin * w.N * w.K;
        break;
      }
      case OP_GEMM: {
        GemmArgs g;
        fill_gemm(u, o, B, g);
        gn_have = 0;
        if (o.gn_next >= 0 && oi + 1 < n_ops) {
          const Ten& to = u->tens[o.out];
          g.gn_part = u->small; g.gn_HW = to.rows; g.gn_G = u->ops[o.gn_next].groups; g.gn_done = &gn_have;
        }
        if (o.glu_op >= 0 && o.glu_op < n_ops) {
          const Op& ge = u->ops[o.glu_op];
          g.glu_y = u->aptr(ge.out); g.glu_ldy = u->tens[ge.out].ld;
          if (!save) g.C = nullptr;
        }
        u->flops_fwd += launch_gemm(dt, g, st);
        break;
      }
      case OP_GN: {
        const Ten& t = u->tens[o.in0];
        const int have = (oi > 0 && u->ops[oi - 1].gn_next == oi) ? gn_have : 0;
        launch_groupnorm_fwd(dt, u->aptr(o.in0), u->pf + o.gamma_off, u->pf + o.beta_off, u->aptr(o.out),
                             u->f32a + o.stats_off, u->small, B, t.rows, t.C, o.groups, o.eps, o.silu, st, have);
        gn_have = 0;
        break;
      }
      case OP_LN: {
        if (o.folded && use_ln_fold(u, B)) break;
        const Ten& t = u->tens[o.in0];
        launch_layernorm_fwd(dt, u->aptr(o.in0), u->pf + (o.folded ? u->ones_off : o.gamma_off),
                             u->pf + (o.folded ? u->zeros_off : o.beta_off), u->aptr(o.out),
                             u->f32a + o.stats_off, B * t.rows, t.C, o.eps, st, t.ld);
        break;
      }
      case OP_ATTN: {
        const Ten& tq = u->tens[o.in0];
        const int C = u->tens[o.out].C;
        if (!o.cross) {
          const unsigned short* qkv = u->aptr(o.in0);
          launch_attention_fwd(dt, qkv, tq.C, qkv + C, qkv + 2 * C, tq.C, u->aptr(o.out), C, u->f32a + o.lse_off, B,
                               o.heads, o.Nq, o.Nk, st);
        } else {
          const Ten& tkv = u->tens[o.in1];
          const unsigned short* kv = u->aptr(o.in1) + o.kv_col;
          launch_attention_fwd(dt, u->aptr(o.in0), tq.C, kv, kv + C, tkv.C, u->aptr(o.out), C, u->f32a + o.lse_off, B,
                               o.heads, o.Nq, o.Nk, st);
        }
        u->flops_fwd += 4.0 * B * o.heads * (double)o.Nq * o.Nk * 64;
        break;
      }
      case OP_GEGLU: {
        if (oi > 0 && u->ops[oi - 1].glu_op == oi) break;
        const Ten& t = u->tens[o.out];
        launch_geglu_fwd(dt, u->aptr(o.in0), u->aptr(o.out), B * t.rows, t.C, st);
        break;
      }
      case OP_CONCAT: {
        const Ten &a = u->tens[o.in0], &b2 = u->tens[o.in1], &t = u->tens[o.out];
        gn_have = 0;
        const int G = o.gn_next >= 0 ? u->ops[o.gn_next].groups : 0;
        if (o.gn_next >= 0 && oi + 1 < n_ops && a.C % 8 == 0 && b2.C % 8 == 0 && t.C % G == 0 &&
            (GN_GB * (t.C / G)) % 8 == 0 && GN_GB * (t.C / G) <= 2048) {
          launch_concat_gn(dt, u->aptr(o.in0), a.C, u->aptr(o.in1), b2.C, u->aptr(o.out), u->small, B, t.rows, G, st);
          gn_have = 1;
        } else {
          launch_copy_cols(dt, u->aptr(o.in0), a.C, u->aptr(o.out), t.C, B * t.rows, a.C, 0, st);
          launch_copy_cols(dt, u->aptr(o.in1), b2.C, u->aptr(o.out) + a.C, t.C, B * t.rows, b2.C, 0, st);
        }
        break;
      }
    }
  }
}

static uint64_t graph_key_fwd(int B, int n_ops, bool temb_hit, bool kv_hit, bool save) {
  return (uint64_t)B | ((uint64_t)n_ops << 12) | ((uint64_t)(temb_hit ? 1 : 0) << 34) | ((uint64_t)(kv_hit ? 1 : 0) << 36) |
         ((uint64_t)(save ? 1 : 0) << 37);
}
static uint64_t graph_key_bwd(int B, unsigned mask, bool eps, bool sample, bool text) {
  return (uint64_t)B | ((uint64_t)(mask & 7u) << 28) | ((uint64_t)(eps ? 1 : 0) << 31) | ((uint64_t)(sample ? 1 : 0) << 32) |
         ((uint64_t)(text ? 1 : 0) << 33) | (1ull << 35);
}

template <class F>
static int run_graphed(dh_unet* u, uint64_t key, hipStream_t st, double* flops_slot, F body) {
  if (!u->use_graphs || st == nullptr || gemm_profiling_on()) { body(); return DH_OK; }
  auto it = u->graphs.find(key);
  if (it == u->graphs.end()) {
    hipGraph_t graph = nullptr;
    DH_CHECK_HIP(hipStreamBeginCapture(st, hipStreamCaptureModeThreadLocal));
    body();
    DH_CHECK_HIP(hipStreamEndCapture(st, &graph));
    hipGraphExec_t exec = nullptr;
    DH_CHECK_HIP(hipGraphInstantiate(&exec, graph, nullptr, nullptr, 0));
    (void)hipGraphDestroy(graph);
    u->graphs[key] = exec;
    u->graph_flops[key] = *flops_slot;
    it = u->graphs.find(key);
  }
  *flops_slot = u->graph_flops[key];
// ... 180 lines not shown
          if (oi > 0 && u->ops[oi - 1].type == OP_GN && u->ops[oi - 1].out == o.in0) gi = oi - 1;
          else if (oi > 1 && u->ops[oi - 1].type == OP_GEMM && u->ops[oi - 1].mode == A_DENSE && u->ops[oi - 1].out == o.res &&
                   u->ops[oi - 1].in0 != o.in0 && u->ops[oi - 2].type == OP_GN && u->ops[oi - 2].out == o.in0)
            gi = oi - 2;
          if (gi >= 0) {
            const Op& gn = u->ops[gi];
            const Ten& tx = u->tens[gn.in0];
            g.gnb_x = u->aptr(gn.in0); g.gnb_ldx = tx.ld;
            g.gnb_gamma = u->pf + gn.gamma_off; g.gnb_beta = u->pf + gn.beta_off; g.gnb_stats = u->f32a + gn.stats_off;
            g.gnb_silu = gn.silu;
            g.gn_part = u->small; g.gn_HW = tx.rows; g.gn_G = gn.groups; g.gn_done = &gnb_have;
            gnb_for = gi;
          }
          u->flops_bwd += launch_gemm(dt, g, st);
          u->gready[o.in0] = 1;
        }
        if (o.in0 == u->t_text) text_grad_written = true;
        break;
      }
      case OP_GN: {
        if (!u->gready[o.out]) break;
        const Ten& t = u->tens[o.in0];
        GnBwdSplit split;
        if (oi > 0 && u->ops[oi - 1].type == OP_CONCAT && u->ops[oi - 1].out == o.in0) {
          const Op& cat = u->ops[oi - 1];
          const int ca = u->tens[cat.in0].C;
          if (!u->gready[cat.in0] && !u->gready[cat.in1] && ca % 8 == 0 && ca + u->tens[cat.in1].C == t.C) {
            split.out0 = u->gptr(cat.in0); split.out1 = u->gptr(cat.in1); split.split_c = ca;
            cat_done = oi - 1;
          }
        }
        launch_groupnorm_bwd(dt, u->aptr(o.in0), u->gptr(o.out), u->pf + o.gamma_off, u->pf + o.beta_off,
                             u->f32a + o.stats_off, u->gptr(o.in0), u->small, B, t.rows, t.C, o.groups, o.silu,
                             u->gready[o.in0] ? 1 : 0, st, gnb_for == oi ? gnb_have : 0, split);
        gnb_have = 0;
        u->gready[o.in0] = 1;
        if (split.out0) { u->gready[u->ops[oi - 1].in0] = 1; u->gready[u->ops[oi - 1].in1] = 1; }
        break;
      }
      case OP_LN: {
        if (!u->gready[o.out]) break;
        if (lnb_have && lnb_for == oi) {
          lnb_have = 0;
          u->gready[o.in0] = 1;
          break;
        }
        const Ten& t = u->tens[o.in0];
        launch_layernorm_bwd(dt, u->aptr(o.in0), u->gptr(o.out), u->pf + o.gamma_off, u->f32a + o.stats_off,
                             u->gready[o.in0] ? u->gptr(o.in0) : nullptr, u->gptr(o.in0), B * t.rows, t.C, st, t.ld);
        u->gready[o.in0] = 1;
        break;
      }
      case OP_GEGLU: {
        if (!u->gready[o.out]) break;
        if (glub_done == oi) { glub_done = -1; break; }
        const Ten& t = u->tens[o.out];
        launch_geglu_bwd(dt, u->aptr(o.in0), u->gptr(o.out), u->gptr(o.in0), B * t.rows, t.C, st);
        u->gready[o.in0] = 1;
        break;
      }
      case OP_ATTN: {
        if (!u->gready[o.out]) break;
        const Ten& tq = u->tens[o.in0];
        const int C = u->tens[o.out].C;
        float* delta = u->small;
        if (!o.cross) {
          const unsigned short* qkv = u->aptr(o.in0);
// ... 160 lines not shown
```

diffusionhandles_amd/csrc/unet_kernels.h:

```cpp
#pragma once
#include "common.h"

namespace dh {

__device__ inline float silu_grad(float z) {
  const float s = 1.f / (1.f + __expf(-z));
  return s * (1.f + z * (1.f - s));
}

struct GeluParts { float Phi, pdf; };
__device__ __forceinline__ GeluParts gelu_parts(float g) {
  const float x = fabsf(g) * 0.70710678118654752f;
  const float t = __builtin_amdgcn_rcpf(fmaf(0.3275911f, x, 1.f));
  const float e = __expf(-x * x);
  const float poly = t * (0.254829592f + t * (-0.284496736f + t * (1.421413741f + t * (-1.453152027f + t * 1.061405429f))));
  const float q = 0.5f * poly * e;
  return {g < 0.f ? q : 1.f - q, e * 0.3989422804014327f};
}
__device__ __forceinline__ float gelu_f(float g) { return g * gelu_parts(g).Phi; }
__device__ __forceinline__ float gelu_grad(float g) { const GeluParts p = gelu_parts(g); return fmaf(g, p.pdf, p.Phi); }
__host__ __device__ inline int glu_col(int o, int gate) { return 32 * (o >> 4) + 16 * gate + (o & 15); }
__host__ __device__ inline int glu_src_row(int n, int F) { return ((n >> 4) & 1) * F + 16 * (n >> 5) + (n & 15); }

enum { A_DENSE = 0, A_CONV3 = 1, A_CONVT2 = 2 };

struct GemmArgs {
  const void* A = nullptr; long lda = 0;
  const void* W = nullptr;
  int M = 0, N = 0, K = 0;
  int mode = A_DENSE;
  int Hin = 0, Win = 0, Cin = 0;
  int Hout = 0, Wout = 0;
  int stride = 1, up = 0;
  int pad = 1;
  const float* bias = nullptr;
  const float* rowvec = nullptr; int rowvec_ld = 0; int rows_per_batch = 1;
  const void* R = nullptr; long ldr = 0;
  void* C = nullptr; long ldc = 0;
  int act_silu = 0;
  float* partial = nullptr; size_t partial_elems = 0;
  float* gn_part = nullptr; int gn_HW = 0, gn_G = 0; int* gn_done = nullptr;
  const void* gnb_x = nullptr; long gnb_ldx = 0; const float *gnb_gamma = nullptr, *gnb_beta = nullptr, *gnb_stats = nullptr;
  int gnb_silu = 0;
  const float* ln_s = nullptr; const float* ln_t = nullptr; float* ln_stats = nullptr; float ln_eps = 1e-5f;
  const void* lnb_x = nullptr; long lnb_ldx = 0; const float *lnb_gamma = nullptr, *lnb_stats = nullptr; const void* lnb_add = nullptr;
  void* lnb_dx = nullptr; int* lnb_done = nullptr;
  void* glu_y = nullptr; long glu_ldy = 0;
  const void* glub_x = nullptr; void* glub_dx = nullptr; int glub_f = 0;
};
void launch_splitk_reduce_ln_bwd(int dtype, const float* partial, int splits, const void* x, const float* gamma,
                                 const float* stats, const void* add, void* dx, int rows, int C, hipStream_t st, long ldx = 0);
double launch_gemm(int dtype, const GemmArgs& a, hipStream_t st);
bool gemm_profiling_on();
void launch_tile_weights(int dtype, const void* src, void* dst, int N, int K, hipStream_t st, int conv_cin = 0);
__host__ __device__ inline size_t wt_index(int n, int k, int K) {
  const int r = n & 63, c = (k & 63) >> 3;
  return ((size_t)(n >> 6) * (K >> 6) + (k >> 6)) * 4096 + (size_t)r * 64 + (size_t)((c ^ ((r >> 1) & 7)) << 3) + (k & 7);
}

__host__ __device__ inline int conv_k_index(int tap, int c) { return (c >> 6) * 576 + tap * 64 + (c & 63); }

void launch_load_weight(int dtype, const float* src, int N, int C, int taps, void* fwd, long fwd_K, long row_off, void* bwd,
                        long bwd_K, long col_off, int Nb, float scale, hipStream_t st);

void launch_conv_small_fwd(int dtype, const void* x, int x_is_f32, const float* w, const float* bias, void* y,
                           int y_is_f32, int B, int H, int W, int Cin, int Cout, hipStream_t st);
void launch_conv_small_bwd(int dtype, const void* dy, int dy_is_f32, const float* w, void* dx, int dx_is_f32,
                           int accumulate, int B, int H, int W, int Cin, int Cout, hipStream_t st);

void launch_groupnorm_fwd(int dtype, const void* x, const float* gamma, const float* beta, void* y, float* stats,
                          float* scratch, int B, int HW, int C, int G, float eps, int silu, hipStream_t st,
                          int have_partials = 0);
int gn_slices(int HW, int B);
constexpr int GN_GB = 4;
void launch_concat_gn(int dtype, const void* a, int Ca, const void* b, int Cb, void* out, float* gn_part, int B, int HW,
                      int G, hipStream_t st);
struct GnBwdSplit { void* out0 = nullptr; void* out1 = nullptr; int split_c = 0; };
void launch_groupnorm_bwd(int dtype, const void* x, const void* dy, const float* gamma, const float* beta,
                          const float* stats, void* dx, float* scratch, int B, int HW, int C, int G, int silu,
                          int accumulate, hipStream_t st, int have_partials = 0, GnBwdSplit split = GnBwdSplit());
void launch_gelu(int dtype, const void* x, void* y, size_t n, hipStream_t st);
void launch_layernorm_fwd(int dtype, const void* x, const float* gamma, const float* beta, void* y, float* stats,
                          int rows, int C, float eps, hipStream_t st, long ldx = 0);
void launch_layernorm_bwd(int dtype, const void* x, const void* dy, const float* gamma, const float* stats,
                          const void* add, void* dx, int rows, int C, hipStream_t st, long ldx = 0);
void launch_geglu_fwd(int dtype, const void* x, void* y, int rows, int F, hipStream_t st);
void launch_geglu_bwd(int dtype, const void* x, const void* dy, void* dx, int rows, int F, hipStream_t st);
void launch_copy_cols(int dtype, const void* src, long lds, void* dst, long ldd, int rows, int cols, int accumulate,
                      hipStream_t st);
void launch_split_cols(int dtype, const void* src, long lds, void* dstA, long ldA, int colsA, int accA, void* dstB, long ldB,
                       int colsB, int accB, int rows, hipStream_t st);
void launch_lane_ops_probe(const float* in, float* out, unsigned* ex, hipStream_t st);
void launch_pool2x2_sum(int dtype, const void* src, void* dst, int B, int h, int w, int C, int accumulate,
                        hipStream_t st);
void launch_f32_to_t(int dtype, const float* src, void* dst, size_t n, hipStream_t st);
void launch_t_to_f32(int dtype, const void* src, float* dst, size_t n, int accumulate, hipStream_t st);
void launch_timestep_embedding(int dtype, const float* t_dev, int dim, int B, void* out, hipStream_t st);
void launch_set_scalar(float* p, float v, hipStream_t st);

void launch_attention_fwd(int dtype, const void* q, long ldq, const void* k, const void* v, long ldk, void* o,
                          long ldo, float* lse, int B, int H, int Nq, int Nk, hipStream_t st, int causal = 0);
void launch_attention_delta(int dtype, const void* o, long ldo, const void* d_o, long lddo, float* delta, int B,
                            int H, int Nq, hipStream_t st);
void launch_attention_bwd_dq(int dtype, const void* q, long ldq, const void* k, const void* v, long ldk, const void* o,
                             long ldo, const void* d_o, long lddo, const float* lse, float* delta, void* dq, long lddq,
                             int B, int H, int Nq, int Nk, hipStream_t st);
void launch_attention_bwd_dkv(int dtype, const void* q, long ldq, const void* k, const void* v, long ldk,
                              const void* d_o, long lddo, const float* lse, const float* delta, void* dk, void* dv,
                              long lddk, int B, int H, int Nq, int Nk, hipStream_t st, float* scratch = nullptr,
                              size_t scratch_elems = 0);

}
```

diffusionhandles_amd/csrc/unet_kernels.hip:

```cpp
#include "unet_kernels.h"

namespace dh {

#ifdef DH_TUNING
static int ablate_mask() { static const int m = getenv("DH_ABLATE_SKIP") ? atoi(getenv("DH_ABLATE_SKIP")) : 0; return m; }
__global__ void k_noop() {}
static int ablate_empty() { static const int m = getenv("DH_ABLATE_EMPTY") ? atoi(getenv("DH_ABLATE_EMPTY")) : 0; return m; }
#define DH_ABLATE(bit) do { if (ablate_mask() & (bit)) { if (ablate_empty()) hipLaunchKernelGGL(k_noop, dim3(1), dim3(64), 0, st); return; } } while (0)
#else
#define DH_ABLATE(bit) do { } while (0)
#endif

constexpr int CF_PIX = 4;
template <class T>
__global__ void k_conv_few_in(const float* x, const float* w, const float* bias, T* y, int B, int H, int W, int Ci,
                              int Co) {
  __shared__ float patch[CF_PIX][9 * 8];
  const int K = 9 * Ci, total = B * H * W;
  const int p0 = blockIdx.x * CF_PIX;
  for (int i = threadIdx.x; i < CF_PIX * K; i += blockDim.x) {
    const int lp = i / K, k = i - lp * K, p = p0 + lp;
    float v = 0.f;
    if (p < total) {
      const int b = p / (H * W), r = p - b * H * W, oy = r / W, ox = r - oy * W;
// ... 92 lines not shown
      hipLaunchKernelGGL((k_conv_few_out<bf16>), dim3(conv_few_out_blocks(B * H * W, Cin)), dim3(256), 0, st, (const bf16*)x, w, bias, (float*)y, B, H, W, Cin, Cout, 0);
  }
}

void launch_conv_small_bwd(int dtype, const void* dy, int dy_is_f32, const float* w, void* dx, int dx_is_f32,
                           int accumulate, int B, int H, int W, int Cin, int Cout, hipStream_t st) {
  if (dy_is_f32) {
    if (dtype == DH_DTYPE_F16)
      hipLaunchKernelGGL((k_conv_few_in<f16>), dim3(cdiv(B * H * W, CF_PIX)), dim3(256), 0, st, (const float*)dy, w, (const float*)nullptr, (f16*)dx, B, H, W, Cin, Cout);
    else
      hipLaunchKernelGGL((k_conv_few_in<bf16>), dim3(cdiv(B * H * W, CF_PIX)), dim3(256), 0, st, (const float*)dy, w, (const float*)nullptr, (bf16*)dx, B, H, W, Cin, Cout);
  } else {
    if (!conv_few_out_ok(Cin, Cout, w)) return;
    if (dtype == DH_DTYPE_F16)
      hipLaunchKernelGGL((k_conv_few_out<f16>), dim3(conv_few_out_blocks(B * H * W, Cin)), dim3(256), 0, st, (const f16*)dy, w, (const float*)nullptr, (float*)dx, B, H, W, Cin, Cout, accumulate);
    else
      hipLaunchKernelGGL((k_conv_few_out<bf16>), dim3(conv_few_out_blocks(B * H * W, Cin)), dim3(256), 0, st, (const bf16*)dy, w, (const float*)nullptr, (float*)dx, B, H, W, Cin, Cout, accumulate);
  }
}

__device__ __forceinline__ float silu_f(float z) { return z / (1.f + __expf(-z)); }

static int gn_slice_cap(int B) {
#ifdef DH_TUNING
  static const int v = getenv("DH_GN_SLICES") ? atoi(getenv("DH_GN_SLICES")) : 0;
  if (v > 0) return v > 64 ? 64 : v;
#endif
  return B <= 2 ? 32 : 16;
}
int gn_slices(int HW, int B) { const int cap = gn_slice_cap(B); int s = HW / 4; return s < 1 ? 1 : (s > cap ? cap : s); }

template <class T, bool BWD>
__global__ void __launch_bounds__(256) k_gn_partial(const T* x, const T* dy, const float* gamma, const float* beta,
                                                    const float* stats, float* part, int HW, int C, int G, int S, int silu) {
  __shared__ float sm_red[4][2 * GN_GB];
  const int s = blockIdx.x, g0 = blockIdx.y * GN_GB, b = blockIdx.z, cpg = div_small(C, rcp_fast(G));
  const int W = GN_GB * cpg, nch = W >> 3;
  const float inv_nch = rcp_fast(nch), inv_S = rcp_fast(S);
  const int RP = div_small((int)blockDim.x, inv_nch);
  const int r0 = div_small(HW * s, inv_S), r1 = div_small(HW * (s + 1), inv_S);
  const size_t base = (size_t)b * HW * C + (size_t)g0 * cpg;
  const int rr = div_small((int)threadIdx.x, inv_nch), ch = threadIdx.x - rr * nch;
  float ga[GN_GB], gq[GN_GB], pg[GN_GB];
#pragma unroll
  for (int gl = 0; gl < GN_GB; ++gl) {
    ga[gl] = 0.f; gq[gl] = 0.f;
    pg[gl] = (BWD || g0 + gl >= G) ? 0.f : to_f32<T>(x[base + (size_t)r0 * C + gl * cpg]);
  }
  if (rr < RP) {
    int gi[8];
    const float inv_cpg = rcp_fast(cpg);
    float a[8], q[8], pv[8], gm[8], bt[8], mu[8], rs[8];
#pragma unroll
    for (int i = 0; i < 8; ++i) {
      gi[i] = div_small(ch * 8 + i, inv_cpg);
      a[i] = 0.f; q[i] = 0.f; pv[i] = 0.f;
#pragma unroll
      for (int gl = 0; gl < GN_GB; ++gl) pv[i] = gi[i] == gl ? pg[gl] : pv[i];
    }
    if (BWD) {
      *reinterpret_cast<float4*>(gm) = *reinterpret_cast<const float4*>(gamma + g0 * cpg + ch * 8);
      *reinterpret_cast<float4*>(gm + 4) = *reinterpret_cast<const float4*>(gamma + g0 * cpg + ch * 8 + 4);
      *reinterpret_cast<float4*>(bt) = *reinterpret_cast<const float4*>(beta + g0 * cpg + ch * 8);
      *reinterpret_cast<float4*>(bt + 4) = *reinterpret_cast<const float4*>(beta + g0 * cpg + ch * 8 + 4);
      float2 st4[GN_GB];
#pragma unroll
      for (int gl = 0; gl < GN_GB; ++gl)
        st4[gl] = g0 + gl < G ? *reinterpret_cast<const float2*>(stats + 2 * (b * G + g0 + gl)) : make_float2(0.f, 0.f);
#pragma unroll
      for (int i = 0; i < 8; ++i) {
        mu[i] = 0.f; rs[i] = 0.f;
#pragma unroll
        for (int gl = 0; gl < GN_GB; ++gl) { mu[i] = gi[i] == gl ? st4[gl].x : mu[i]; rs[i] = gi[i] == gl ? st4[gl].y : rs[i]; }
      }
    }
    for (int r = r0 + rr; r < r1; r += RP) {
      uint4 raw = *reinterpret_cast<const uint4*>(x + base + (size_t)r * C + ch * 8);
      const T* v = reinterpret_cast<const T*>(&raw);
      if (!BWD) {
#pragma unroll
        for (int i = 0; i < 8; ++i) { const float d = to_f32<T>(v[i]) - pv[i]; a[i] += d; q[i] += d * d; }
      } else {
        uint4 rawd = *reinterpret_cast<const uint4*>(dy + base + (size_t)r * C + ch * 8);
        const T* dv = reinterpret_cast<const T*>(&rawd);
#pragma unroll
        for (int i = 0; i < 8; ++i) {
          const float xh = (to_f32<T>(v[i]) - mu[i]) * rs[i];
          float d = to_f32<T>(dv[i]);
          if (silu) d *= silu_grad(xh * gm[i] + bt[i]);
          d *= gm[i];
          a[i] += d;
          q[i] += d * xh;
        }
      }
    }
#pragma unroll
    for (int i = 0; i < 8; ++i)
#pragma unroll
      for (int gl = 0; gl < GN_GB; ++gl) {
        ga[gl] += gi[i] == gl ? a[i] : 0.f;
        gq[gl] += gi[i] == gl ? q[i] : 0.f;
      }
  }
#pragma unroll
  for (int gl = 0; gl < GN_GB; ++gl) { ga[gl] = wave_sum(ga[gl]); gq[gl] = wave_sum(gq[gl]); }
  if ((threadIdx.x & 63) == 0) {
#pragma unroll
    for (int gl = 0; gl < GN_GB; ++gl) { sm_red[threadIdx.x >> 6][2 * gl] = ga[gl]; sm_red[threadIdx.x >> 6][2 * gl + 1] = gq[gl]; }
  }
  __syncthreads();
// ... 22 lines not shown
  const bool act = g < G;
  const float* p = part + ((size_t)(b * G + (act ? g : 0)) * 3) * S;
  float cn[GN_COMBINE_K], cm[GN_COMBINE_K], cq[GN_COMBINE_K];
#pragma unroll
  for (int k = 0; k < GN_COMBINE_K; ++k) {
    const int s = sub + 8 * k;
    const bool on = act && s < S;
    cn[k] = on ? p[s] : 0.f;
    cm[k] = on ? p[S + s] : 0.f;
    cq[k] = on ? p[2 * S + s] : 0.f;
  }
  const float ref = act ? p[S] : 0.f;
  float n = 0.f, sm = 0.f;
#pragma unroll
  for (int k = 0; k < GN_COMBINE_K; ++k) { n += cn[k]; sm += cn[k] * (cm[k] - ref); }
  n = oct_sum(n); sm = oct_sum(sm);
  const float mean = ref + sm / n;
  float m2 = 0.f;
#pragma unroll
  for (int k = 0; k < GN_COMBINE_K; ++k) { const float d = cm[k] - mean; m2 += cq[k] + cn[k] * d * d; }
  m2 = oct_sum(m2);
  m2 = m2 > 0.f ? m2 : 0.f;
  if (act && sub == 0) {
    const float rstd = rsqrtf(m2 / n + eps);
    sm_stats[g] = make_float2(mean, rstd);
    if (stats_out) { stats_out[2 * (b * G + g)] = mean; stats_out[2 * (b * G + g) + 1] = rstd; }
  }
  __syncthreads();
}

template <class T, bool WIDE>
__global__ void __launch_bounds__(256) k_gn_apply(const T* x, const float* gamma, const float* beta, const float* part,
                                                  float* stats, T* y, int HW, int C, int G, int S, float eps, int silu,
                                                  int iters) {
  __shared__ float2 sm_stats[64];
  const int b = blockIdx.y;
  const int cchunks = C / 8, cpg = C / G;
  const float inv_cpg = 1.f / (float)cpg;
  const unsigned total = (unsigned)HW * cchunks;
  unsigned idx = blockIdx.x * iters * blockDim.x + threadIdx.x;
  bool live = idx < total;
  unsigned pix = live ? idx / cchunks : 0;
  size_t row = (size_t)b * HW + pix;
  int c0 = (int)(idx - pix * cchunks) * 8;
  uint4 raw = *reinterpret_cast<const uint4*>(x + row * C + c0);
  float gmv[8], btv[8];
  *reinterpret_cast<float4*>(gmv) = *reinterpret_cast<const float4*>(gamma + c0);
  *reinterpret_cast<float4*>(gmv + 4) = *reinterpret_cast<const float4*>(gamma + c0 + 4);
  *reinterpret_cast<float4*>(btv) = *reinterpret_cast<const float4*>(beta + c0);
  *reinterpret_cast<float4*>(btv + 4) = *reinterpret_cast<const float4*>(beta + c0 + 4);
  gn_combine(part, b, G, S, eps, sm_stats, blockIdx.x == 0 ? stats : nullptr);
  for (int it = 0; it < iters; ++it) {
    if (!live) return;
    uint4 nraw = raw;
    float ngm[8], nbt[8];
    const unsigned nidx = idx + blockDim.x;
    const bool nlive = it + 1 < iters && nidx < total;
    size_t nrow = row;
    int nc0 = c0;
    if (nlive) {
      const unsigned npix = nidx / cchunks;
      nrow = (size_t)b * HW + npix;
      nc0 = (int)(nidx - npix * cchunks) * 8;
      nraw = *reinterpret_cast<const uint4*>(x + nrow * C + nc0);
      *reinterpret_cast<float4*>(ngm) = *reinterpret_cast<const float4*>(gamma + nc0);
      *reinterpret_cast<float4*>(ngm + 4) = *reinterpret_cast<const float4*>(gamma + nc0 + 4);
      *reinterpret_cast<float4*>(nbt) = *reinterpret_cast<const float4*>(beta + nc0);
      *reinterpret_cast<float4*>(nbt + 4) = *reinterpret_cast<const float4*>(beta + nc0 + 4);
    }
    typedef T T8 __attribute__((ext_vector_type(8)));
    const T8 xv = __builtin_bit_cast(T8, raw);
    T8 o;
    const int g0 = (int)(((float)c0 + 0.5f) * inv_cpg), bnd = (g0 + 1) * cpg - c0;
    const float2 st0 = sm_stats[g0], st1 = sm_stats[g0 + 1 < G ? g0 + 1 : g0];
#pragma unroll
    for (int i = 0; i < 8; ++i) {
      const float2 st = WIDE ? (i < bnd ? st0 : st1) : sm_stats[(c0 + i) / cpg];
      float z = (to_f32<T>(xv[i]) - st.x) * st.y * gmv[i] + btv[i];
      if (silu) z = silu_f(z);
      o[i] = from_f32<T>(z);
    }
    *reinterpret_cast<uint4*>(y + row * C + c0) = __builtin_bit_cast(uint4, o);
    if (!nlive) return;
    idx = nidx; row = nrow; c0 = nc0; raw = nraw;
#pragma unroll
    for (int i = 0; i < 8; ++i) { gmv[i] = ngm[i]; btv[i] = nbt[i]; }
  }
}

static inline int gn_apply_iters(size_t blocks_total) {
  size_t it = blocks_total / 1024;
  return it < 1 ? 1 : (it > 8 ? 8 : (int)it);
}

void launch_groupnorm_fwd(int dtype, const void* x, const float* gamma, const float* beta, void* y, float* stats,
                          float* scratch, int B, int HW, int C, int G, float eps, int silu, hipStream_t st,
                          int have_partials) {
  DH_ABLATE(2);
  const int S = have_partials > 1 ? have_partials : gn_slices(HW, B);
  const size_t blocks0 = ((size_t)HW * (C / 8) + 255) / 256;
  const int iters = gn_apply_iters(blocks0 * B);
  dim3 g1(S, cdiv(G, GN_GB), B), g2((unsigned)((blocks0 + iters - 1) / iters), B);
  if (dtype == DH_DTYPE_F16) {
    if (!have_partials) hipLaunchKernelGGL((k_gn_partial<f16, false>), g1, dim3(256), 0, st, (const f16*)x, (const f16*)nullptr, gamma, beta, (const float*)nullptr, scratch, HW, C, G, S, silu);
    if (C / G >= 8) hipLaunchKernelGGL((k_gn_apply<f16, true>), g2, dim3(256), 0, st, (const f16*)x, gamma, beta, scratch, stats, (f16*)y, HW, C, G, S, eps, silu, iters);
    else hipLaunchKernelGGL((k_gn_apply<f16, false>), g2, dim3(256), 0, st, (const f16*)x, gamma, beta, scratch, stats, (f16*)y, HW, C, G, S, eps, silu, iters);
  } else {
    if (!have_partials) hipLaunchKernelGGL((k_gn_partial<bf16, false>), g1, dim3(256), 0, st, (const bf16*)x, (const bf16*)nullptr, gamma, beta, (const float*)nullptr, scratch, HW, C, G, S, silu);
    if (C / G >= 8) hipLaunchKernelGGL((k_gn_apply<bf16, true>), g2, dim3(256), 0, st, (const bf16*)x, gamma, beta, scratch, stats, (bf16*)y, HW, C, G, S, eps, silu, iters);
    else hipLaunchKernelGGL((k_gn_apply<bf16, false>), g2, dim3(256), 0, st, (const bf16*)x, gamma, beta, scratch, stats, (bf16*)y, HW, C, G, S, eps, silu, iters);
  }
}

template <class T, bool WIDE>
__global__ void __launch_bounds__(256) k_gn_bwd_apply(const T* x, const T* dy, const float* gamma, const float* beta,
                                                      const float* stats, const float* part, T* dx, int HW, int C, int G,
                                                      int S, int silu, int accumulate, int iters, T* split0, T* split1,
                                                      int split_c) {
  __shared__ float4 sm_st[64];
  const int b = blockIdx.y, cpg = C / G;
  const float inv_cpg = 1.f / (float)cpg;
  const int cchunks = C / 8;
  const unsigned total = (unsigned)HW * cchunks;
  unsigned idx = blockIdx.x * iters * blockDim.x + threadIdx.x;
  bool live = idx < total;
  unsigned pix = live ? idx / cchunks : 0;
  size_t row = (size_t)b * HW + pix;
  int c0 = (int)(idx - pix * cchunks) * 8;
  uint4 rx = *reinterpret_cast<const uint4*>(x + row * C + c0);
  uint4 rd = *reinterpret_cast<const uint4*>(dy + row * C + c0);
  uint4 ro = make_uint4(0, 0, 0, 0);
  if (accumulate) ro = *reinterpret_cast<const uint4*>(dx + row * C + c0);
  float gmv[8], btv[8];
  *reinterpret_cast<float4*>(gmv) = *reinterpret_cast<const float4*>(gamma + c0);
  *reinterpret_cast<float4*>(gmv + 4) = *reinterpret_cast<const float4*>(gamma + c0 + 4);
  *reinterpret_cast<float4*>(btv) = *reinterpret_cast<const float4*>(beta + c0);
  *reinterpret_cast<float4*>(btv + 4) = *reinterpret_cast<const float4*>(beta + c0 + 4);
  {
    const int g = threadIdx.x >> 3, sub = threadIdx.x & 7;
    const bool act = g < G;
    const float2* p = reinterpret_cast<const float2*>(part) + (size_t)(b * G + (act ? g : 0)) * S;
    float2 v[GN_COMBINE_K];
#pragma unroll
    for (int k = 0; k < GN_COMBINE_K; ++k) {
      const int s = sub + 8 * k;
      v[k] = act && s < S ? p[s] : make_float2(0.f, 0.f);
    }
    float2 st = act ? *reinterpret_cast<const float2*>(stats + 2 * (b * G + g)) : make_float2(0.f, 0.f);
    float a = 0.f, c = 0.f;
#pragma unroll
    for (int k = 0; k < GN_COMBINE_K; ++k) { a += v[k].x; c += v[k].y; }
    a = oct_sum(a); c = oct_sum(c);
    const float inv = 1.f / ((float)HW * (float)cpg);
    if (act && sub == 0) sm_st[g] = make_float4(st.x, st.y, a * inv, c * inv);
  }
  __syncthreads();
  typedef T T8 __attribute__((ext_vector_type(8)));
  for (int it = 0; it < iters; ++it) {
    if (!live) return;
    const unsigned nidx = idx + blockDim.x;
    const bool nlive = it + 1 < iters && nidx < total;
    size_t nrow = row;
    int nc0 = c0;
    uint4 nrx = rx, nrd = rd, nro = ro;
    float ngm[8], nbt[8];
    if (nlive) {
      const unsigned npix = nidx / cchunks;
      nrow = (size_t)b * HW + npix;
      nc0 = (int)(nidx - npix * cchunks) * 8;
      nrx = *reinterpret_cast<const uint4*>(x + nrow * C + nc0);
      nrd = *reinterpret_cast<const uint4*>(dy + nrow * C + nc0);
      if (accumulate) nro = *reinterpret_cast<const uint4*>(dx + nrow * C + nc0);
      *reinterpret_cast<float4*>(ngm) = *reinterpret_cast<const float4*>(gamma + nc0);
      *reinterpret_cast<float4*>(ngm + 4) = *reinterpret_cast<const float4*>(gamma + nc0 + 4);
      *reinterpret_cast<float4*>(nbt) = *reinterpret_cast<const float4*>(beta + nc0);
      *reinterpret_cast<float4*>(nbt + 4) = *reinterpret_cast<const float4*>(beta + nc0 + 4);
    }
    const T8 xv = __builtin_bit_cast(T8, rx), dv = __builtin_bit_cast(T8, rd), ov = __builtin_bit_cast(T8, ro);
    T8 o;
    const int g0 = (int)(((float)c0 + 0.5f) * inv_cpg), bnd = (g0 + 1) * cpg - c0;
    const float4 st0 = sm_st[g0], st1 = sm_st[g0 + 1 < G ? g0 + 1 : g0];
#pragma unroll
    for (int i = 0; i < 8; ++i) {
      const float4 st = WIDE ? (i < bnd ? st0 : st1) : sm_st[(c0 + i) / cpg];
      const float xh = (to_f32<T>(xv[i]) - st.x) * st.y;
      float d = to_f32<T>(dv[i]);
      if (silu) d *= silu_grad(xh * gmv[i] + btv[i]);
      d *= gmv[i];
      float r = st.y * (d - st.z - xh * st.w);
      if (accumulate) r += to_f32<T>(ov[i]);
      o[i] = from_f32<T>(r);
    }
    T* dst = !split0 ? dx + row * C + c0
                     : (c0 < split_c ? split0 + row * split_c + c0 : split1 + row * (C - split_c) + (c0 - split_c));
    *reinterpret_cast<uint4*>(dst) = __builtin_bit_cast(uint4, o);
    if (!nlive) return;
    idx = nidx; row = nrow; c0 = nc0; rx = nrx; rd = nrd; ro = nro;
#pragma unroll
    for (int i = 0; i < 8; ++i) { gmv[i] = ngm[i]; btv[i] = nbt[i]; }
  }
}

void launch_groupnorm_bwd(int dtype, const void* x, const void* dy, const float* gamma, const float* beta,
                          const float* stats, void* dx, float* scratch, int B, int HW, int C, int G, int silu,
                          int accumulate, hipStream_t st, int have_partials, GnBwdSplit split) {
  DH_ABLATE(2);
  const int S = have_partials > 1 ? have_partials : gn_slices(HW, B);
  const size_t blocks0 = ((size_t)HW * (C / 8) + 255) / 256;
  const int iters = gn_apply_iters(blocks0 * B);
  dim3 g1(S, cdiv(G, GN_GB), B), g2((unsigned)((blocks0 + iters - 1) / iters), B);
  if (dtype == DH_DTYPE_F16) {
    if (!have_partials) hipLaunchKernelGGL((k_gn_partial<f16, true>), g1, dim3(256), 0, st, (const f16*)x, (const f16*)dy, gamma, beta, stats, scratch, HW, C, G, S, silu);
    if (C / G >= 8) hipLaunchKernelGGL((k_gn_bwd_apply<f16, true>), g2, dim3(256), 0, st, (const f16*)x, (const f16*)dy, gamma, beta, stats, scratch, (f16*)dx, HW, C, G, S, silu, accumulate, iters, (f16*)split.out0, (f16*)split.out1, split.split_c);
    else hipLaunchKernelGGL((k_gn_bwd_apply<f16, false>), g2, dim3(256), 0, st, (const f16*)x, (const f16*)dy, gamma, beta, stats, scratch, (f16*)dx, HW, C, G, S, silu, accumulate, iters, (f16*)split.out0, (f16*)split.out1, split.split_c);
  } else {
    if (!have_partials) hipLaunchKernelGGL((k_gn_partial<bf16, true>), g1, dim3(256), 0, st, (const bf16*)x, (const bf16*)dy, gamma, beta, stats, scratch, HW, C, G, S, silu);
    if (C / G >= 8) hipLaunchKernelGGL((k_gn_bwd_apply<bf16, true>), g2, dim3(256), 0, st, (const bf16*)x, (const bf16*)dy, gamma, beta, stats, scratch, (bf16*)dx, HW, C, G, S, silu, accumulate, iters, (bf16*)split.out0, (bf16*)split.out1, split.split_c);
    else hipLaunchKernelGGL((k_gn_bwd_apply<bf16, false>), g2, dim3(256), 0, st, (const bf16*)x, (const bf16*)dy, gamma, beta, stats, scratch, (bf16*)dx, HW, C, G, S, silu, accumulate, iters, (bf16*)split.out0, (bf16*)split.out1, split.split_c);
  }
}

template <class T>
__global__ void __launch_bounds__(256) k_concat_gn(const T* a, int Ca, const T* bsrc, int Cb, T* out, float* part, int HW, int G,
                                                   int S) {
  __shared__ float sm_red[4][2 * GN_GB];
  const int C = Ca + Cb;
  const int s = blockIdx.x, g0 = blockIdx.y * GN_GB, b = blockIdx.z, cpg = div_small(C, rcp_fast(G));
  const int W = GN_GB * cpg, nch = W >> 3;
  const float inv_nch = rcp_fast(nch), inv_S = rcp_fast(S);
  const int RP = div_small((int)blockDim.x, inv_nch);
  const int r0 = div_small(HW * s, inv_S), r1 = div_small(HW * (s + 1), inv_S);
  const int rr = div_small((int)threadIdx.x, inv_nch), ch = threadIdx.x - rr * nch;
  auto load8 = [&](size_t m, int n) {
    return n < Ca ? *reinterpret_cast<const uint4*>(a + m * Ca + n) : *reinterpret_cast<const uint4*>(bsrc + m * Cb + (n - Ca));
  };
  float ga[GN_GB], gq[GN_GB], pg[GN_GB];
#pragma unroll
  for (int gl = 0; gl < GN_GB; ++gl) {
    ga[gl] = 0.f; gq[gl] = 0.f; pg[gl] = 0.f;
    if (g0 + gl < G) {
      const int n = (g0 + gl) * cpg;
      const size_t m = (size_t)b * HW + r0;
      pg[gl] = to_f32<T>(n < Ca ? a[m * Ca + n] : bsrc[m * Cb + (n - Ca)]);
    }
  }
  if (rr < RP && g0 * cpg + ch * 8 < C) {
    const int n = g0 * cpg + ch * 8;
    int gi[8];
    const float inv_cpg = rcp_fast(cpg);
    float av[8], qv[8], pv[8];
#pragma unroll
    for (int i = 0; i < 8; ++i) {
      gi[i] = div_small(ch * 8 + i, inv_cpg);
      av[i] = 0.f; qv[i] = 0.f; pv[i] = 0.f;
#pragma unroll
      for (int gl = 0; gl < GN_GB; ++gl) pv[i] = gi[i] == gl ? pg[gl] : pv[i];
    }
    for (int r = r0 + rr; r < r1; r += RP) {
      const size_t m = (size_t)b * HW + r;
      const uint4 raw = load8(m, n);
      *reinterpret_cast<uint4*>(out + m * C + n) = raw;
      const T* v = reinterpret_cast<const T*>(&raw);
#pragma unroll
      for (int i = 0; i < 8; ++i) { const float d = to_f32<T>(v[i]) - pv[i]; av[i] += d; qv[i] += d * d; }
    }
#pragma unroll
    for (int i = 0; i < 8; ++i)
#pragma unroll
      for (int gl = 0; gl < GN_GB; ++gl) {
        ga[gl] += gi[i] == gl ? av[i] : 0.f;
        gq[gl] += gi[i] == gl ? qv[i] : 0.f;
      }
  }
#pragma unroll
  for (int gl = 0; gl < GN_GB; ++gl) { ga[gl] = wave_sum(ga[gl]); gq[gl] = wave_sum(gq[gl]); }
  if ((threadIdx.x & 63) == 0) {
#pragma unroll
    for (int gl = 0; gl < GN_GB; ++gl) { sm_red[threadIdx.x >> 6][2 * gl] = ga[gl]; sm_red[threadIdx.x >> 6][2 * gl + 1] = gq[gl]; }
  }
  __syncthreads();
  if ((int)threadIdx.x < GN_GB && g0 + (int)threadIdx.x < G) {
    const int gl = threadIdx.x, g = g0 + gl;
    float sa = 0.f, sq = 0.f;
    for (int w = 0; w < 4; ++w) { sa += sm_red[w][2 * gl]; sq += sm_red[w][2 * gl + 1]; }
    const float n = (float)(r1 - r0) * (float)cpg;
    float piv = 0.f;
#pragma unroll
    for (int k = 0; k < GN_GB; ++k) piv = gl == k ? pg[k] : piv;
    float* o = part + ((size_t)(b * G + g) * 3) * S + s;
    o[0] = n; o[S] = piv + sa / n; o[2 * S] = sq - sa * sa / n;
  }
}

void launch_concat_gn(int dtype, const void* a, int Ca, const void* b, int Cb, void* out, float* gn_part, int B, int HW,
                      int G, hipStream_t st) {
  DH_ABLATE(8);
  const int S = gn_slices(HW, B);
  dim3 grid(S, cdiv(G, GN_GB), B);
  if (dtype == DH_DTYPE_F16)
    hipLaunchKernelGGL((k_concat_gn<f16>), grid, dim3(256), 0, st, (const f16*)a, Ca, (const f16*)b, Cb, (f16*)out, gn_part, HW, G, S);
  else
    hipLaunchKernelGGL((k_concat_gn<bf16>), grid, dim3(256), 0, st, (const bf16*)a, Ca, (const bf16*)b, Cb, (bf16*)out, gn_part, HW, G, S);
}

constexpr int LN_MAXCH = 8;

template <class T, int NCH>
__global__ void __launch_bounds__(256, NCH <= 3 ? 4 : 1) k_ln_fwd(const T* x, const float* gamma, const float* beta, T* y, float* stats, int rows, int C,
                         float eps, long ldx) {
  const int lane = threadIdx.x & 63;
  const int row = blockIdx.x * (blockDim.x >> 6) + (threadIdx.x >> 6);
  if (row >= rows) return;
  const int nch = C / 8;
  uint4 raw[NCH];
  float s = 0.f;
#pragma unroll
  for (int k = 0; k < NCH; ++k) {
    const int ch = lane + 64 * k;
    if (ch < nch) {
      raw[k] = *reinterpret_cast<const uint4*>(x + (size_t)row * ldx + ch * 8);
      const T* v = reinterpret_cast<const T*>(&raw[k]);
#pragma unroll
      for (int i = 0; i < 8; ++i) s += to_f32<T>(v[i]);
    }
  }
  const float mean = wave_sum(s) / (float)C;
  float q = 0.f;
#pragma unroll
  for (int k = 0; k < NCH; ++k) {
    const int ch = lane + 64 * k;
    if (ch < nch) {
      const T* v = reinterpret_cast<const T*>(&raw[k]);
#pragma unroll
      for (int i = 0; i < 8; ++i) { const float d = to_f32<T>(v[i]) - mean; q += d * d; }
    }
// ... 459 lines not shown
```

Measured before the change: 36.30 steps/s.

## Fold resnet 1x1 shortcut GEMM into conv2 via concatenated K dimension

For resnet blocks whose input and output channel counts differ, the 1x1 conv_shortcut is folded into the conv2 implicit GEMM. The input x is laid out in a shared buffer next to the norm2 output, and the shortcut weights are appended as extra K columns after the nine 3x3 taps. The two biases are pre-summed. A conv cursor walks the 9*c9 tap tiles and then the centre-tap-only tail. This removes a separate GEMM launch and the write and re-read of its result as the residual, at the cost of strided tensor views and added cursor logic in the GEMM kernels and groupnorm/concat kernels.

```diff
diff --git a/diffusionhandles_amd/_lib.py b/diffusionhandles_amd/_lib.py
--- a/diffusionhandles_amd/_lib.py
+++ b/diffusionhandles_amd/_lib.py
@@ -126,7 +126,10 @@
     "dh_dbg_gemm_groupnorm_bwd_res": (c_i, [c_i, c_p, c_l, c_p, c_i, c_i, c_i, c_i, c_i, c_i, c_i, c_p, c_l, c_p, c_p, c_sz, c_i, c_i, c_p, c_p, c_p,
                                         c_p, c_i, c_p, c_p, ctypes.POINTER(c_i), c_p]),
     "dh_dbg_concat_groupnorm": (c_i, [c_i, c_p, c_i, c_p, c_i, c_p, c_i, c_i, c_i, c_p, c_p, c_f, c_i, c_p, c_p, c_p, c_p]),
+    "dh_dbg_gemm_conv_sc_groupnorm": (c_i, [c_i, c_p, c_l, c_p, c_i, c_i, c_i, c_i, c_i, c_i, c_p, c_p, c_p, c_sz, c_i, c_i, c_p, c_p,
+                                             c_f, c_i, c_p, c_p, c_p, ctypes.POINTER(c_i), c_p]),
     "dh_dbg_gemm_last_tile": (c_i, [ctypes.POINTER(c_i)]),
+    "dh_dbg_conv_cursor": (c_i, [c_i, c_i, c_i, c_i, ctypes.POINTER(c_i), ctypes.POINTER(c_i)]),
     "dh_dbg_unet_concat_ops": (c_i, [ctypes.POINTER(UNetConfig), ctypes.POINTER(c_i), c_i, ctypes.POINTER(c_i)]),
     "dh_dbg_gemm_lnfold": (c_i, [c_i, c_p, c_l, c_p, c_i, c_i, c_i, c_p, c_p, c_p, c_f, c_p, c_l, c_p]),
     "dh_dbg_gemm_glu": (c_i, [c_i, c_i, c_p, c_l, c_p, c_i, c_i, c_i, c_p, c_p, c_p, c_p, c_p, c_p]),
diff --git a/diffusionhandles_amd/csrc/debug_api.cpp b/diffusionhandles_amd/csrc/debug_api.cpp
--- a/diffusionhandles_amd/csrc/debug_api.cpp
+++ b/diffusionhandles_amd/csrc/debug_api.cpp
@@ -76,6 +76,34 @@
                                      int* have_out, void* stream) {
   return dh_dbg_gemm_groupnorm_res(dtype, A, lda, W, M, N, K, mode, Hin, Win, Cin, bias, nullptr, N, C, partial, partial_elems, HW, G,
                                    gamma, beta, eps, silu, Y, stats, scratch, have_out, stream);
+}
+extern "C" int dh_dbg_gemm_conv_sc_groupnorm(int dtype, const void* A, long lda, const void* W, int M, int N, int c9, int Cx, int Hin, int Win,
+                                             const float* bias, void* C, float* partial, size_t partial_elems, int HW, int G,
+                                             const float* gamma, const float* beta, float eps, int silu, void* Y, float* stats,
+                                             float* scratch, int* have_out, void* stream) {
+  DH_REQUIRE(A && W && C && Y && stats && scratch && gamma && beta && c9 > 0 && c9 % 64 == 0 && Cx > 0 && Cx % 64 == 0 && N % 64 == 0 &&
+             lda >= c9 + Cx && HW > 0 && M % HW == 0 && HW == Hin * Win, "bad arguments");
+  static void* tiled = nullptr;
+  static size_t cap = 0;
+  const int K = 9 * c9 + Cx;
+  const size_t need = (size_t)N * K * 2;
+  if (need > cap) {
+    if (tiled) (void)hipFree(tiled);
+    DH_CHECK_HIP(hipMalloc(&tiled, need));
+    cap = need;
+  }
+  launch_tile_weights(dtype, W, tiled, N, K, (hipStream_t)stream, c9);
+  GemmArgs g;
+  g.A = A; g.lda = lda; g.W = tiled; g.M = M; g.N = N; g.K = K; g.mode = A_CONV3; g.Hin = Hin; g.Win = Win; g.Cin = c9 + Cx; g.c9 = c9;
+  g.Hout = Hin; g.Wout = Win; g.stride = 1; g.up = 0; g.bias = bias; g.C = C; g.ldc = N;
+  g.partial = partial; g.partial_elems = partial_elems;
+  int have = 0;
+  g.gn_part = scratch; g.gn_HW = HW; g.gn_G = G; g.gn_done = &have;
+  launch_gemm(dtype, g, (hipStream_t)stream);
+  launch_groupnorm_fwd(dtype, C, gamma, beta, Y, stats, scratch, M / HW, HW, N, G, eps, silu, (hipStream_t)stream, have);
+  if (have_out) *have_out = have;
+  DH_LAUNCH_CHECK();
+  return DH_OK;
 }
 extern "C" int dh_dbg_gemm_groupnorm_bwd_res(int dtype, const void* A, long lda, const void* W, int M, int N, int K, int mode, int Hin,
                                          int Win, int Cin, const void* R, long ldr, void* C, float* partial, size_t partial_elems, int HW, int G, const void* x,
diff --git a/diffusionhandles_amd/csrc/gemm.hip b/diffusionhandles_amd/csrc/gemm.hip
--- a/diffusionhandles_amd/csrc/gemm.hip
+++ b/diffusionhandles_amd/csrc/gemm.hip
@@ -99,13 +99,16 @@
 }
 
 typedef int buf_v4i __attribute__((ext_vector_type(4)));
+#pragma clang diagnostic push
+#pragma clang diagnostic ignored "-Winline-asm"
 __device__ __forceinline__ void buf_dma16(unsigned voff, buf_v4i rsrc, unsigned soff, unsigned lds_dst) {
   unsigned tmp;
   soff = __builtin_amdgcn_readfirstlane(soff);
   lds_dst = __builtin_amdgcn_readfirstlane(lds_dst);
   asm volatile("s_mov_b32 m0, %4\n\ts_mov_b32 %0, %3\n\tbuffer_load_dwordx4 %1, %2, %0 offen lds"
-               : "=&s"(tmp) : "v"(voff), "s"(rsrc), "s"(soff), "s"(lds_dst) : "memory");
-}
+               : "=&s"(tmp) : "v"(voff), "s"(rsrc), "s"(soff), "s"(lds_dst) : "memory", "m0");
+}
+#pragma clang diagnostic pop
 __device__ __forceinline__ unsigned buf_mask_oob(unsigned nt, unsigned sh, unsigned voff) {
   return ((nt << sh) & 0x80000000u) | voff;
 }
@@ -240,7 +243,7 @@
     b_ptr[j] = Wg + ((size_t)((n0 + row) >> 6) * KT) * 4096 + (size_t)((n0 + row) & 63) * 64 + lane * 8;
   }
   int tap = 0, c0 = 0;
-  if (MODE != GM_DENSE) { const int kt0 = kbeg >> 6, ch = kt0 / 9; tap = kt0 - ch * 9; c0 = ch * BK; }
+  if (MODE != GM_DENSE) conv_cursor_at(kbeg >> 6, p.c9, tap, c0);
   typedef int bv4i __attribute__((ext_vector_type(4)));
   bv4i ra = {0, 0, 0, 0}, rw = {0, 0, 0, 0};
   unsigned bv_a[NPA], bv_nt[NPA], bs_w[NPB];
@@ -336,15 +339,19 @@
   };
   auto next_tile = [&]() {
     if constexpr (BUF && MODE == GM_CONV_S1) {
-      ++tap; ++bs_kx;
+      ++bs_kx;
       const bool row_end = bs_kx == 3;
       bs_tap += row_end ? bs_step_row : bs_step_px;
       bs_kx = row_end ? 0 : bs_kx;
-      if (tap == 9) { tap = 0; c0 += BK; bs_tap = (unsigned)c0 * 2u; }
+      if (conv_cursor_next(p.c9, tap, c0)) {
+        const int ky = tap == 4 ? 1 : 0;
+        bs_tap = (unsigned)((ky * p.Win + ky) * (int)p.lda + c0) * 2u;
+        bs_kx = ky;
+      }
       bs_sh = 31u - (unsigned)tap;
       return;
     }
-    if (MODE != GM_DENSE) { if (++tap == 9) { tap = 0; c0 += BK; } }
+    if (MODE != GM_DENSE) conv_cursor_next(p.c9, tap, c0);
   };
   auto issue = [&](int kt, int stage) {
 #pragma unroll
@@ -902,7 +909,7 @@
   if (idx >= (size_t)N * K) return;
   const int n = (int)(idx / K);
   int k = (int)(idx - (size_t)n * K);
-  if (conv_cin) { const int tap = k / conv_cin; k = conv_k_index(tap, k - tap * conv_cin); }
+  if (conv_cin && k < 9 * conv_cin) { const int tap = k / conv_cin; k = conv_k_index(tap, k - tap * conv_cin); }
   dst[wt_index(n, k, K)] = src[idx];
 }
 void launch_tile_weights(int dtype, const void* src, void* dst, int N, int K, hipStream_t st, int conv_cin) {
@@ -1263,7 +1270,7 @@
     else if (k.Hout > 0 && k.Wout > 0 && k.M % (k.Hout * k.Wout) == 0)
       ab = (size_t)(k.M / (k.Hout * k.Wout)) * k.Hin * k.Win * (size_t)k.lda * 2;
     const size_t wb = (size_t)align_up((size_t)k.N, 64) * k.K * 2;
-    const bool conv_ok = k.mode == A_DENSE || (k.Cin % 64 == 0 && k.K == 9 * k.Cin);
+    const bool conv_ok = k.mode == A_DENSE || (k.Cin % 64 == 0 && k.c9 % 64 == 0 && k.K == BK * conv_k_tiles(k.Cin, k.c9));
     if ((g_buf_stage & 1) && ab > 0 && conv_ok && ab + (size_t)(k.Win + 1) * k.lda * 2 < 0x7ff00000ull && wb < 0x7ff00000ull && k.lda % 8 == 0 &&
         ((size_t)k.A & 15) == 0 && ((size_t)k.W & 15) == 0) {
       k.pp_a_bytes = (unsigned)ab; k.pp_w_bytes = (unsigned)wb;
@@ -1326,6 +1333,7 @@
   k.A = a.A; k.lda = a.lda; k.W = a.W; k.M = a.M; k.N = a.N; k.K = a.K;
   k.mode = a.mode; k.Hin = a.Hin; k.Win = a.Win; k.Cin = a.Cin; k.Hout = a.Hout; k.Wout = a.Wout;
   k.stride = a.stride; k.up = a.up; k.pad = a.pad;
+  k.c9 = a.c9 > 0 ? a.c9 : a.Cin;
   k.bias = a.bias; k.rowvec = a.rowvec; k.rowvec_ld = a.rowvec_ld;
   k.rows_per_batch = a.rows_per_batch > 0 ? a.rows_per_batch : 1;
   k.inv_rows_per_batch = 1.f / (float)k.rows_per_batch;
@@ -1379,6 +1387,18 @@
   return DH_OK;
 }
 
+extern "C" int dh_dbg_conv_cursor(int Cin, int c9, int kt0, int n, int* out, int* tiles) {
+  DH_REQUIRE(out && tiles && Cin > 0 && Cin % 64 == 0 && c9 > 0 && c9 % 64 == 0 && c9 <= Cin && kt0 >= 0 && n >= 0, "bad arguments");
+  *tiles = dh::conv_k_tiles(Cin, c9);
+  int tap = 0, c0 = 0;
+  dh::conv_cursor_at(kt0, c9, tap, c0);
+  for (int i = 0; i < n; ++i) {
+    out[2 * i] = tap; out[2 * i + 1] = c0;
+    dh::conv_cursor_next(c9, tap, c0);
+  }
+  return DH_OK;
+}
+
 extern "C" int dh_gemm_profile_begin(void) {
   dh::g_prof.on = true;
   dh::g_prof.used = 0;
diff --git a/diffusionhandles_amd/csrc/gemm_k.h b/diffusionhandles_amd/csrc/gemm_k.h
--- a/diffusionhandles_amd/csrc/gemm_k.h
+++ b/diffusionhandles_amd/csrc/gemm_k.h
@@ -24,6 +24,7 @@
   const void* W;
   int M, N, K;
   int mode, Hin, Win, Cin, Hout, Wout, stride, up, pad;
+  int c9;
   const float* bias;
   const float* rowvec; int rowvec_ld; int rows_per_batch; float inv_rows_per_batch;
   const void* R; long ldr;
@@ -53,6 +54,20 @@
 __host__ __device__ constexpr bool glub_tile_is_glu(int n0, int glub_f) { return n0 < glub_f; }
 __host__ __device__ constexpr bool glub_split_ok(int BN, int glub_f) { return BN > 0 && glub_f % BN == 0; }
 
+__host__ __device__ constexpr int conv_k_tiles(int Cin, int c9) { return (c9 >> 6) * 9 + ((Cin - c9) >> 6); }
+__host__ __device__ inline void conv_cursor_at(int kt0, int c9, int& tap, int& c0) {
+  const int n9 = (c9 >> 6) * 9;
+  if (kt0 < n9) { const int ch = kt0 / 9; tap = kt0 - ch * 9; c0 = ch * 64; }
+  else { tap = 4; c0 = c9 + (kt0 - n9) * 64; }
+}
+__host__ __device__ inline bool conv_cursor_next(int c9, int& tap, int& c0) {
+  if (c0 >= c9) { c0 += 64; return true; }
+  if (++tap < 9) return false;
+  c0 += 64;
+  tap = c0 >= c9 ? 4 : 0;
+  return true;
+}
+
 struct PpPlan { int bm = 0, bn = 0, splits = 1; };
 bool gemm_pp_plan(const GemmK& k, size_t partial_elems, int force, PpPlan* plan);
 void launch_gemm_pp(int dtype, const GemmK& k, const PpPlan& plan, hipStream_t st, hipEvent_t e0, hipEvent_t e1);
diff --git a/diffusionhandles_amd/csrc/gemm_pp.hip b/diffusionhandles_amd/csrc/gemm_pp.hip
--- a/diffusionhandles_amd/csrc/gemm_pp.hip
+++ b/diffusionhandles_amd/csrc/gemm_pp.hip
@@ -150,7 +150,7 @@
     w_soff[j] = (unsigned)(((n >> 6) * KT) * 8192 + (n & 63) * 128) + (unsigned)(kbeg >> 6) * 8192u - 1024u * j;
   }
   int tap = 0, c0 = 0;
-  if (MODE != PP_DENSE) { const int kt0 = kbeg >> 6, ch = kt0 / 9; tap = kt0 - ch * 9; c0 = ch * 64; }
+  if (MODE != PP_DENSE) conv_cursor_at(kbeg >> 6, p.c9, tap, c0);
   int kt_issue = 0;
   int kti = 0;
   int issued = 0;
@@ -206,7 +206,7 @@
   auto next_tile = [&]() {
     ++kt_issue;
     kti = __builtin_amdgcn_readfirstlane(kt_issue);
-    if (MODE != PP_DENSE) { if (++tap == 9) { tap = 0; c0 += 64; } }
+    if (MODE != PP_DENSE) conv_cursor_next(p.c9, tap, c0);
   };
   int rpre_n = 0;
   auto wait_tile = [&](int u) {
@@ -583,7 +583,7 @@
   if (k.bias && ((size_t)k.bias & 15)) return false;
   if ((k.C && (k.ldc % 8 || ((size_t)k.C & 15))) || k.lda % 8 || ((size_t)k.A & 15) || ((size_t)k.W & 15)) return false;
   if (k.R && (k.ldr % 8 || ((size_t)k.R & 15))) return false;
-  if (k.mode != A_DENSE && (k.Hout <= 0 || k.Wout <= 0 || k.M % (k.Hout * k.Wout) || k.Cin % 64 || k.K != 9 * k.Cin)) return false;
+  if (k.mode != A_DENSE && (k.Hout <= 0 || k.Wout <= 0 || k.M % (k.Hout * k.Wout) || k.Cin % 64 || k.c9 % 64 || k.K != 64 * conv_k_tiles(k.Cin, k.c9))) return false;
   const size_t ab = pp_a_bytes(k) + (size_t)(k.Win + 1) * k.lda * 2, wb = (size_t)k.N * k.K * 2;
   if (ab >= 0x7ff00000ull || wb >= 0x7ff00000ull) return false;
   const int ktiles = k.K / 64;
@@ -696,7 +696,7 @@
   dh::GemmK k{};
   k.A = dummy; k.W = dummy; k.C = dummy; k.M = M; k.N = N; k.K = K; k.lda = conv ? K / 9 : K; k.ldc = N;
   k.mode = conv ? dh::A_CONV3 : dh::A_DENSE;
-  if (conv) { k.Hin = k.Win = k.Hout = k.Wout = hw; k.Cin = K / 9; k.stride = 1; k.up = 0; k.pad = 1; }
+  if (conv) { k.Hin = k.Win = k.Hout = k.Wout = hw; k.Cin = K / 9; k.c9 = k.Cin; k.stride = 1; k.up = 0; k.pad = 1; }
   k.partial = partial_elems ? reinterpret_cast<float*>(dummy) : nullptr;
   if (glu == 1) { k.glu_y = dummy; k.glu_ldy = N / 2; }
   if (glu == 2) { k.glub_x = dummy; k.glub_dx = dummy; k.C = nullptr; }
diff --git a/diffusionhandles_amd/csrc/unet_engine.cpp b/diffusionhandles_amd/csrc/unet_engine.cpp
--- a/diffusionhandles_amd/csrc/unet_engine.cpp
+++ b/diffusionhandles_amd/csrc/unet_engine.cpp
@@ -38,6 +38,7 @@
   int wt = -1;
   int row_off = 0;
   int glu_F = 0;
+  int fold_wt = -1, fold_k0 = 0;
 };
 
 struct Op {
@@ -56,11 +57,17 @@
   int ln_fold = -1, folded = 0;
   long ln_s_off = -1, ln_t_off = -1;
   int glu_op = -1, glub_op = -1;
+  int sc_op = -1, sc_folded = 0;
 };
 
 struct FfFold {
   int wt_po = -1, wt_ffo = -1, wt = -1;
   long b_po = -1, b_ffo = -1, bias = -1;
+};
+
+struct ScFold {
+  long b_conv2 = -1, b_sc = -1, bias = -1;
+  int n = 0;
 };
 
 }
@@ -75,6 +82,7 @@
   std::vector<ParamInfo> params;
   std::vector<Op> ops;
   std::vector<FfFold> ffolds;
+  std::vector<ScFold> scfolds;
   std::map<std::string, int> pindex;
   size_t w16_elems = 0, pf_elems = 0, act_elems = 0, grad_elems = 0, f32_elems = 0;
   size_t fo_elems = 0;
@@ -195,14 +203,14 @@
     u.ops.push_back(o);
     return o.out;
   }
-  int conv3(int x, const std::string& pre, int Cout, int Hs, int stride, int up, long temb_off, int res) {
+  int conv3(int x, const std::string& pre, int Cout, int Hs, int stride, int up, long temb_off, int res, int tail = 0) {
     const Ten& tx = u.tens[x];
     const int Cin = tx.C;
     const int Hv = Hs << up, Ho = stride == 2 ? Hv / 2 : Hv;
     Op o;
     o.type = OP_GEMM; o.mode = A_CONV3; o.in0 = x; o.res = res;
     o.Hin = Hs; o.Win = Hs; o.Cin = Cin; o.Hout = Ho; o.Wout = Ho; o.stride = stride; o.up = up;
-    o.wt = weight(Cout, 9 * Cin, 9);
+    o.wt = weight(Cout, 9 * Cin + tail, 9);
     bind_mat(pre + ".weight", o.wt, Cout, 0, Cin, 9);
     o.bias_off = param_f32(pre + ".bias", Cout);
     if (temb_off >= 0) { o.rowvec_off = u.temb_f32_off + temb_off; o.rowvec_ld = u.temb_total; }
@@ -252,6 +260,9 @@
 
   int resnet(int x, const std::string& pre, int Cout, int H) {
     const int Cin = u.tens[x].C;
+    const bool fold = Cin != Cout && Cin % 64 == 0 && Cout % 64 == 0 && u.tens[x].view < 0;
+    int cat = -1;
+    if (fold) { cat = tensor(u.tens[x].rows, Cout + Cin, false); set_view(x, cat, Cout); }
     int h = gn(x, pre + ".norm1", 1e-5f, true);
     bind_mat(pre + ".time_emb_proj.weight", wt_temb, Cout, temb_cursor, u.cfg.block_out_channels[0] * 4, 1);
     param_f32_at(pre + ".time_emb_proj.bias", Cout, temb_bias_off + temb_cursor);
@@ -259,9 +270,24 @@
     temb_cursor += Cout;
     h = conv3(h, pre + ".conv1", Cout, H, 1, 0, toff, -1);
     h = gn(h, pre + ".norm2", 1e-5f, true);
+    if (fold) set_view(h, cat, 0);
     int sc = x;
     if (Cin != Cout) sc = linear(x, pre + ".conv_shortcut", Cout, true, -1, true);
-    return conv3(h, pre + ".conv2", Cout, H, 1, 0, -1, sc);
+    const int sc_op = (int)u.ops.size() - 1;
+    const int out = conv3(h, pre + ".conv2", Cout, H, 1, 0, -1, sc, fold ? Cin : 0);
+    if (fold) {
+      Op& c2 = u.ops.back();
+      Op& so = u.ops[sc_op];
+      so.sc_folded = 1; c2.sc_op = sc_op;
+      ParamInfo& pw = u.params[u.pindex[pre + ".conv_shortcut.weight"]];
+      pw.fold_wt = c2.wt; pw.fold_k0 = 9 * Cout;
+      ScFold f;
+      f.b_conv2 = c2.bias_off; f.b_sc = so.bias_off; f.n = Cout;
+      f.bias = (long)u.pf_elems; u.pf_elems += align_up((size_t)Cout, 64);
+      c2.bias_off = f.bias;
+      u.scfolds.push_back(f);
+    }
+    return out;
   }
 
   int transformer(int x, const std::string& pre, int heads, int H) {
@@ -472,7 +498,8 @@
   auto wr = [&](int t, int oi) { t = root(t); if (t >= 0) { first[t] = std::min(first[t], oi); last[t] = std::max(last[t], oi); } };
   for (int oi = 0; oi < nops; ++oi) {
     const Op& o = u.ops[oi];
-    rd(o.in0, oi); rd(o.in1, oi); rd(o.res, oi); wr(o.out, oi);
+    if (o.sc_folded) continue;
+    rd(o.in0, oi); rd(o.in1, oi); if (o.sc_op < 0) rd(o.res, oi); wr(o.out, oi);
     if (o.ln_fold >= 0) rd(u.ops[o.ln_fold].in0, oi);
     if (o.glu_op >= 0) wr(u.ops[o.glu_op].out, oi);
   }
@@ -547,6 +574,18 @@
   }
 }
 
+template <class D>
+__global__ void k_load_cols(const float* src, int N, int C, D* fwd, int K, int k0) {
+  const size_t idx = (size_t)blockIdx.x * blockDim.x + threadIdx.x;
+  if (idx >= (size_t)N * C) return;
+  const int n = (int)(idx / C), c = (int)(idx - (size_t)n * C);
+  fwd[wt_index(n, k0 + c, K)] = from_f32<D>(src[idx]);
+}
+__global__ void k_add_f32(const float* a, const float* b, float* out, int n) {
+  const int i = blockIdx.x * blockDim.x + threadIdx.x;
+  if (i < n) out[i] = a[i] + b[i];
+}
+
 }
 namespace dh {
 void launch_load_weight(int dtype, const float* src, int N, int C, int taps, void* fwd, long fwd_K, long row_off, void* bwd,
@@ -674,6 +713,8 @@
   }
   if (u->dtype == DH_DTYPE_F16) fold_ff_t<f16>(u, st);
   else fold_ff_t<bf16>(u, st);
+  for (const ScFold& f : u->scfolds)
+    hipLaunchKernelGGL(k_add_f32, dim3(cdiv(f.n, 256)), dim3(256), 0, st, u->pf + f.b_conv2, u->pf + f.b_sc, u->pf + f.bias, f.n);
   u->fold_dirty = false;
 }
 
@@ -830,6 +871,13 @@
     hipLaunchKernelGGL((k_load_weight<bf16, true>), dim3(nb), dim3(256), 0, st, src, N, C, taps, f, fwd_ld, (long)p.row_off, b,
                        bwd_ld, (long)p.row_off, w.N, 1.f, w.glu_F);
   }
+  if (p.fold_wt >= 0) {
+    const Wt& wf = u->wts[p.fold_wt];
+    if (u->dtype == DH_DTYPE_F16)
+      hipLaunchKernelGGL((k_load_cols<f16>), dim3(nb), dim3(256), 0, st, src, N, C, (f16*)(u->w16 + wf.fwd_off), wf.K, p.fold_k0);
+    else
+      hipLaunchKernelGGL((k_load_cols<bf16>), dim3(nb), dim3(256), 0, st, src, N, C, (bf16*)(u->w16 + wf.fwd_off), wf.K, p.fold_k0);
+  }
   DH_LAUNCH_CHECK();
   return DH_OK;
 }
@@ -850,7 +898,8 @@
   g.stride = o.stride; g.up = o.up;
   g.bias = o.bias_off >= 0 ? u->pf + o.bias_off : nullptr;
   if (o.rowvec_off >= 0) { g.rowvec = u->f32a + o.rowvec_off; g.rowvec_ld = o.rowvec_ld; g.rows_per_batch = to.rows; }
-  if (o.res >= 0) { g.R = u->aptr(o.res); g.ldr = u->tens[o.res].ld; }
+  if (o.sc_op >= 0) { g.Cin = ti.ld; g.c9 = o.Cin; }
+  else if (o.res >= 0) { g.R = u->aptr(o.res); g.ldr = u->tens[o.res].ld; }
   g.C = u->aptr(o.out); g.ldc = to.ld;
   g.act_silu = o.act_silu;
   g.partial = u->partial; g.partial_elems = u->partial_elems;
@@ -897,6 +946,7 @@
         break;
       }
       case OP_GEMM: {
+        if (o.sc_folded) break;
         GemmArgs g;
         fill_gemm(u, o, B, g);
         gn_have = 0;
@@ -916,7 +966,8 @@
         const Ten& t = u->tens[o.in0];
         const int have = (oi > 0 && u->ops[oi - 1].gn_next == oi) ? gn_have : 0;
         launch_groupnorm_fwd(dt, u->aptr(o.in0), u->pf + o.gamma_off, u->pf + o.beta_off, u->aptr(o.out),
-                             u->f32a + o.stats_off, u->small, B, t.rows, t.C, o.groups, o.eps, o.silu, st, have);
+                             u->f32a + o.stats_off, u->small, B, t.rows, t.C, o.groups, o.eps, o.silu, st, have, t.ld,
+                             u->tens[o.out].ld);
         gn_have = 0;
         break;
       }
@@ -956,11 +1007,12 @@
         const int G = o.gn_next >= 0 ? u->ops[o.gn_next].groups : 0;
         if (o.gn_next >= 0 && oi + 1 < n_ops && a.C % 8 == 0 && b2.C % 8 == 0 && t.C % G == 0 &&
             (GN_GB * (t.C / G)) % 8 == 0 && GN_GB * (t.C / G) <= 2048) {
-          launch_concat_gn(dt, u->aptr(o.in0), a.C, u->aptr(o.in1), b2.C, u->aptr(o.out), u->small, B, t.rows, G, st);
+          launch_concat_gn(dt, u->aptr(o.in0), a.C, u->aptr(o.in1), b2.C, u->aptr(o.out), u->small, B, t.rows, G, st, a.ld, b2.ld,
+                           t.ld);
           gn_have = 1;
         } else {
-          launch_copy_cols(dt, u->aptr(o.in0), a.C, u->aptr(o.out), t.C, B * t.rows, a.C, 0, st);
-          launch_copy_cols(dt, u->aptr(o.in1), b2.C, u->aptr(o.out) + a.C, t.C, B * t.rows, b2.C, 0, st);
+          launch_copy_cols(dt, u->aptr(o.in0), a.ld, u->aptr(o.out), t.ld, B * t.rows, a.C, 0, st);
+          launch_copy_cols(dt, u->aptr(o.in1), b2.ld, u->aptr(o.out) + a.C, t.ld, B * t.rows, b2.C, 0, st);
         }
         break;
       }
@@ -1207,7 +1259,7 @@
         }
         launch_groupnorm_bwd(dt, u->aptr(o.in0), u->gptr(o.out), u->pf + o.gamma_off, u->pf + o.beta_off,
                              u->f32a + o.stats_off, u->gptr(o.in0), u->small, B, t.rows, t.C, o.groups, o.silu,
-                             u->gready[o.in0] ? 1 : 0, st, gnb_for == oi ? gnb_have : 0, split);
+                             u->gready[o.in0] ? 1 : 0, st, gnb_for == oi ? gnb_have : 0, split, t.ld);
         gnb_have = 0;
         u->gready[o.in0] = 1;
         if (split.out0) { u->gready[u->ops[oi - 1].in0] = 1; u->gready[u->ops[oi - 1].in1] = 1; }
diff --git a/diffusionhandles_amd/csrc/unet_kernels.h b/diffusionhandles_amd/csrc/unet_kernels.h
--- a/diffusionhandles_amd/csrc/unet_kernels.h
+++ b/diffusionhandles_amd/csrc/unet_kernels.h
@@ -32,6 +32,7 @@
   int Hin = 0, Win = 0, Cin = 0;
   int Hout = 0, Wout = 0;
   int stride = 1, up = 0;
+  int c9 = 0;
   int pad = 1;
   const float* bias = nullptr;
   const float* rowvec = nullptr; int rowvec_ld = 0; int rows_per_batch = 1;
@@ -70,15 +71,16 @@
 
 void launch_groupnorm_fwd(int dtype, const void* x, const float* gamma, const float* beta, void* y, float* stats,
                           float* scratch, int B, int HW, int C, int G, float eps, int silu, hipStream_t st,
-                          int have_partials = 0);
+                          int have_partials = 0, long ldx = 0, long ldy = 0);
 int gn_slices(int HW, int B);
 constexpr int GN_GB = 4;
 void launch_concat_gn(int dtype, const void* a, int Ca, const void* b, int Cb, void* out, float* gn_part, int B, int HW,
-                      int G, hipStream_t st);
+                      int G, hipStream_t st, long lda = 0, long ldb = 0, long ldo = 0);
 struct GnBwdSplit { void* out0 = nullptr; void* out1 = nullptr; int split_c = 0; };
 void launch_groupnorm_bwd(int dtype, const void* x, const void* dy, const float* gamma, const float* beta,
                           const float* stats, void* dx, float* scratch, int B, int HW, int C, int G, int silu,
-                          int accumulate, hipStream_t st, int have_partials = 0, GnBwdSplit split = GnBwdSplit());
+                          int accumulate, hipStream_t st, int have_partials = 0, GnBwdSplit split = GnBwdSplit(),
+                          long ldx = 0);
 void launch_gelu(int dtype, const void* x, void* y, size_t n, hipStream_t st);
 void launch_layernorm_fwd(int dtype, const void* x, const float* gamma, const float* beta, void* y, float* stats,
                           int rows, int C, float eps, hipStream_t st, long ldx = 0);
diff --git a/diffusionhandles_amd/csrc/unet_kernels.hip b/diffusionhandles_amd/csrc/unet_kernels.hip
--- a/diffusionhandles_amd/csrc/unet_kernels.hip
+++ b/diffusionhandles_amd/csrc/unet_kernels.hip
@@ -148,7 +148,8 @@
 
 template <class T, bool BWD>
 __global__ void __launch_bounds__(256) k_gn_partial(const T* x, const T* dy, const float* gamma, const float* beta,
-                                                    const float* stats, float* part, int HW, int C, int G, int S, int silu) {
+                                                    const float* stats, float* part, int HW, int C, int G, int S, int silu,
+                                                    long ldx) {
   __shared__ float sm_red[4][2 * GN_GB];
   const int s = blockIdx.x, g0 = blockIdx.y * GN_GB, b = blockIdx.z, cpg = div_small(C, rcp_fast(G));
   const int W = GN_GB * cpg, nch = W >> 3;
@@ -156,12 +157,13 @@
   const int RP = div_small((int)blockDim.x, inv_nch);
   const int r0 = div_small(HW * s, inv_S), r1 = div_small(HW * (s + 1), inv_S);
   const size_t base = (size_t)b * HW * C + (size_t)g0 * cpg;
+  const size_t xbase = (size_t)b * HW * ldx + (size_t)g0 * cpg;
   const int rr = div_small((int)threadIdx.x, inv_nch), ch = threadIdx.x - rr * nch;
   float ga[GN_GB], gq[GN_GB], pg[GN_GB];
 #pragma unroll
   for (int gl = 0; gl < GN_GB; ++gl) {
     ga[gl] = 0.f; gq[gl] = 0.f;
-    pg[gl] = (BWD || g0 + gl >= G) ? 0.f : to_f32<T>(x[base + (size_t)r0 * C + gl * cpg]);
+    pg[gl] = (BWD || g0 + gl >= G) ? 0.f : to_f32<T>(x[xbase + (size_t)r0 * ldx + gl * cpg]);
   }
   if (rr < RP) {
     int gi[8];
@@ -191,7 +193,7 @@
       }
     }
     for (int r = r0 + rr; r < r1; r += RP) {
-      uint4 raw = *reinterpret_cast<const uint4*>(x + base + (size_t)r * C + ch * 8);
+      uint4 raw = *reinterpret_cast<const uint4*>(x + xbase + (size_t)r * ldx + ch * 8);
       const T* v = reinterpret_cast<const T*>(&raw);
       if (!BWD) {
 #pragma unroll
@@ -280,7 +282,7 @@
 template <class T, bool WIDE>
 __global__ void __launch_bounds__(256) k_gn_apply(const T* x, const float* gamma, const float* beta, const float* part,
                                                   float* stats, T* y, int HW, int C, int G, int S, float eps, int silu,
-                                                  int iters) {
+                                                  int iters, long ldx, long ldy) {
   __shared__ float2 sm_stats[64];
   const int b = blockIdx.y;
   const int cchunks = C / 8, cpg = C / G;
@@ -291,7 +293,7 @@
   unsigned pix = live ? idx / cchunks : 0;
   size_t row = (size_t)b * HW + pix;
   int c0 = (int)(idx - pix * cchunks) * 8;
-  uint4 raw = *reinterpret_cast<const uint4*>(x + row * C + c0);
+  uint4 raw = *reinterpret_cast<const uint4*>(x + row * ldx + c0);
   float gmv[8], btv[8];
   *reinterpret_cast<float4*>(gmv) = *reinterpret_cast<const float4*>(gamma + c0);
   *reinterpret_cast<float4*>(gmv + 4) = *reinterpret_cast<const float4*>(gamma + c0 + 4);
@@ -310,7 +312,7 @@
       const unsigned npix = nidx / cchunks;
       nrow = (size_t)b * HW + npix;
       nc0 = (int)(nidx - npix * cchunks) * 8;
-      nraw = *reinterpret_cast<const uint4*>(x + nrow * C + nc0);
+      nraw = *reinterpret_cast<const uint4*>(x + nrow * ldx + nc0);
       *reinterpret_cast<float4*>(ngm) = *reinterpret_cast<const float4*>(gamma + nc0);
       *reinterpret_cast<float4*>(ngm + 4) = *reinterpret_cast<const float4*>(gamma + nc0 + 4);
       *reinterpret_cast<float4*>(nbt) = *reinterpret_cast<const float4*>(beta + nc0);
@@ -328,7 +330,7 @@
       if (silu) z = silu_f(z);
       o[i] = from_f32<T>(z);
     }
-    *reinterpret_cast<uint4*>(y + row * C + c0) = __builtin_bit_cast(uint4, o);
+    *reinterpret_cast<uint4*>(y + row * ldy + c0) = __builtin_bit_cast(uint4, o);
     if (!nlive) return;
     idx = nidx; row = nrow; c0 = nc0; raw = nraw;
 #pragma unroll
@@ -343,20 +345,22 @@
 
 void launch_groupnorm_fwd(int dtype, const void* x, const float* gamma, const float* beta, void* y, float* stats,
                           float* scratch, int B, int HW, int C, int G, float eps, int silu, hipStream_t st,
-                          int have_partials) {
+                          int have_partials, long ldx, long ldy) {
   DH_ABLATE(2);
+  if (ldx <= 0) ldx = C;
+  if (ldy <= 0) ldy = C;
   const int S = have_partials > 1 ? have_partials : gn_slices(HW, B);
   const size_t blocks0 = ((size_t)HW * (C / 8) + 255) / 256;
   const int iters = gn_apply_iters(blocks0 * B);
   dim3 g1(S, cdiv(G, GN_GB), B), g2((unsigned)((blocks0 + iters - 1) / iters), B);
   if (dtype == DH_DTYPE_F16) {
-    if (!have_partials) hipLaunchKernelGGL((k_gn_partial<f16, false>), g1, dim3(256), 0, st, (const f16*)x, (const f16*)nullptr, gamma, beta, (const float*)nullptr, scratch, HW, C, G, S, silu);
-    if (C / G >= 8) hipLaunchKernelGGL((k_gn_apply<f16, true>), g2, dim3(256), 0, st, (const f16*)x, gamma, beta, scratch, stats, (f16*)y, HW, C, G, S, eps, silu, iters);
-    else hipLaunchKernelGGL((k_gn_apply<f16, false>), g2, dim3(256), 0, st, (const f16*)x, gamma, beta, scratch, stats, (f16*)y, HW, C, G, S, eps, silu, iters);
+    if (!have_partials) hipLaunchKernelGGL((k_gn_partial<f16, false>), g1, dim3(256), 0, st, (const f16*)x, (const f16*)nullptr, gamma, beta, (const float*)nullptr, scratch, HW, C, G, S, silu, ldx);
+    if (C / G >= 8) hipLaunchKernelGGL((k_gn_apply<f16, true>), g2, dim3(256), 0, st, (const f16*)x, gamma, beta, scratch, stats, (f16*)y, HW, C, G, S, eps, silu, iters, ldx, ldy);
+    else hipLaunchKernelGGL((k_gn_apply<f16, false>), g2, dim3(256), 0, st, (const f16*)x, gamma, beta, scratch, stats, (f16*)y, HW, C, G, S, eps, silu, iters, ldx, ldy);
   } else {
-    if (!have_partials) hipLaunchKernelGGL((k_gn_partial<bf16, false>), g1, dim3(256), 0, st, (const bf16*)x, (const bf16*)nullptr, gamma, beta, (const float*)nullptr, scratch, HW, C, G, S, silu);
-    if (C / G >= 8) hipLaunchKernelGGL((k_gn_apply<bf16, true>), g2, dim3(256), 0, st, (const bf16*)x, gamma, beta, scratch, stats, (bf16*)y, HW, C, G, S, eps, silu, iters);
-    else hipLaunchKernelGGL((k_gn_apply<bf16, false>), g2, dim3(256), 0, st, (const bf16*)x, gamma, beta, scratch, stats, (bf16*)y, HW, C, G, S, eps, silu, iters);
+    if (!have_partials) hipLaunchKernelGGL((k_gn_partial<bf16, false>), g1, dim3(256), 0, st, (const bf16*)x, (const bf16*)nullptr, gamma, beta, (const float*)nullptr, scratch, HW, C, G, S, silu, ldx);
+    if (C / G >= 8) hipLaunchKernelGGL((k_gn_apply<bf16, true>), g2, dim3(256), 0, st, (const bf16*)x, gamma, beta, scratch, stats, (bf16*)y, HW, C, G, S, eps, silu, iters, ldx, ldy);
+    else hipLaunchKernelGGL((k_gn_apply<bf16, false>), g2, dim3(256), 0, st, (const bf16*)x, gamma, beta, scratch, stats, (bf16*)y, HW, C, G, S, eps, silu, iters, ldx, ldy);
   }
 }
 
@@ -364,7 +368,7 @@
 __global__ void __launch_bounds__(256) k_gn_bwd_apply(const T* x, const T* dy, const float* gamma, const float* beta,
                                                       const float* stats, const float* part, T* dx, int HW, int C, int G,
                                                       int S, int silu, int accumulate, int iters, T* split0, T* split1,
-                                                      int split_c) {
+                                                      int split_c, long ldx) {
   __shared__ float4 sm_st[64];
   const int b = blockIdx.y, cpg = C / G;
   const float inv_cpg = 1.f / (float)cpg;
@@ -375,7 +379,7 @@
   unsigned pix = live ? idx / cchunks : 0;
   size_t row = (size_t)b * HW + pix;
   int c0 = (int)(idx - pix * cchunks) * 8;
-  uint4 rx = *reinterpret_cast<const uint4*>(x + row * C + c0);
+  uint4 rx = *reinterpret_cast<const uint4*>(x + row * ldx + c0);
   uint4 rd = *reinterpret_cast<const uint4*>(dy + row * C + c0);
   uint4 ro = make_uint4(0, 0, 0, 0);
   if (accumulate) ro = *reinterpret_cast<const uint4*>(dx + row * C + c0);
@@ -416,7 +420,7 @@
       const unsigned npix = nidx / cchunks;
       nrow = (size_t)b * HW + npix;
       nc0 = (int)(nidx - npix * cchunks) * 8;
-      nrx = *reinterpret_cast<const uint4*>(x + nrow * C + nc0);
+      nrx = *reinterpret_cast<const uint4*>(x + nrow * ldx + nc0);
       nrd = *reinterpret_cast<const uint4*>(dy + nrow * C + nc0);
       if (accumulate) nro = *reinterpret_cast<const uint4*>(dx + nrow * C + nc0);
       *reinterpret_cast<float4*>(ngm) = *reinterpret_cast<const float4*>(gamma + nc0);
@@ -451,26 +455,27 @@
 
 void launch_groupnorm_bwd(int dtype, const void* x, const void* dy, const float* gamma, const float* beta,
                           const float* stats, void* dx, float* scratch, int B, int HW, int C, int G, int silu,
-                          int accumulate, hipStream_t st, int have_partials, GnBwdSplit split) {
+                          int accumulate, hipStream_t st, int have_partials, GnBwdSplit split, long ldx) {
   DH_ABLATE(2);
+  if (ldx <= 0) ldx = C;
   const int S = have_partials > 1 ? have_partials : gn_slices(HW, B);
   const size_t blocks0 = ((size_t)HW * (C / 8) + 255) / 256;
   const int iters = gn_apply_iters(blocks0 * B);
   dim3 g1(S, cdiv(G, GN_GB), B), g2((unsigned)((blocks0 + iters - 1) / iters), B);
   if (dtype == DH_DTYPE_F16) {
-    if (!have_partials) hipLaunchKernelGGL((k_gn_partial<f16, true>), g1, dim3(256), 0, st, (const f16*)x, (const f16*)dy, gamma, beta, stats, scratch, HW, C, G, S, silu);
-    if (C / G >= 8) hipLaunchKernelGGL((k_gn_bwd_apply<f16, true>), g2, dim3(256), 0, st, (const f16*)x, (const f16*)dy, gamma, beta, stats, scratch, (f16*)dx, HW, C, G, S, silu, accumulate, iters, (f16*)split.out0, (f16*)split.out1, split.split_c);
-    else hipLaunchKernelGGL((k_gn_bwd_apply<f16, false>), g2, dim3(256), 0, st, (const f16*)x, (const f16*)dy, gamma, beta, stats, scratch, (f16*)dx, HW, C, G, S, silu, accumulate, iters, (f16*)split.out0, (f16*)split.out1, split.split_c);
+    if (!have_partials) hipLaunchKernelGGL((k_gn_partial<f16, true>), g1, dim3(256), 0, st, (const f16*)x, (const f16*)dy, gamma, beta, stats, scratch, HW, C, G, S, silu, ldx);
+    if (C / G >= 8) hipLaunchKernelGGL((k_gn_bwd_apply<f16, true>), g2, dim3(256), 0, st, (const f16*)x, (const f16*)dy, gamma, beta, stats, scratch, (f16*)dx, HW, C, G, S, silu, accumulate, iters, (f16*)split.out0, (f16*)split.out1, split.split_c, ldx);
+    else hipLaunchKernelGGL((k_gn_bwd_apply<f16, false>), g2, dim3(256), 0, st, (const f16*)x, (const f16*)dy, gamma, beta, stats, scratch, (f16*)dx, HW, C, G, S, silu, accumulate, iters, (f16*)split.out0, (f16*)split.out1, split.split_c, ldx);
   } else {
-    if (!have_partials) hipLaunchKernelGGL((k_gn_partial<bf16, true>), g1, dim3(256), 0, st, (const bf16*)x, (const bf16*)dy, gamma, beta, stats, scratch, HW, C, G, S, silu);
-    if (C / G >= 8) hipLaunchKernelGGL((k_gn_bwd_apply<bf16, true>), g2, dim3(256), 0, st, (const bf16*)x, (const bf16*)dy, gamma, beta, stats, scratch, (bf16*)dx, HW, C, G, S, silu, accumulate, iters, (bf16*)split.out0, (bf16*)split.out1, split.split_c);
-    else hipLaunchKernelGGL((k_gn_bwd_apply<bf16, false>), g2, dim3(256), 0, st, (const bf16*)x, (const bf16*)dy, gamma, beta, stats, scratch, (bf16*)dx, HW, C, G, S, silu, accumulate, iters, (bf16*)split.out0, (bf16*)split.out1, split.split_c);
+    if (!have_partials) hipLaunchKernelGGL((k_gn_partial<bf16, true>), g1, dim3(256), 0, st, (const bf16*)x, (const bf16*)dy, gamma, beta, stats, scratch, HW, C, G, S, silu, ldx);
+    if (C / G >= 8) hipLaunchKernelGGL((k_gn_bwd_apply<bf16, true>), g2, dim3(256), 0, st, (const bf16*)x, (const bf16*)dy, gamma, beta, stats, scratch, (bf16*)dx, HW, C, G, S, silu, accumulate, iters, (bf16*)split.out0, (bf16*)split.out1, split.split_c, ldx);
+    else hipLaunchKernelGGL((k_gn_bwd_apply<bf16, false>), g2, dim3(256), 0, st, (const bf16*)x, (const bf16*)dy, gamma, beta, stats, scratch, (bf16*)dx, HW, C, G, S, silu, accumulate, iters, (bf16*)split.out0, (bf16*)split.out1, split.split_c, ldx);
   }
 }
 
 template <class T>
 __global__ void __launch_bounds__(256) k_concat_gn(const T* a, int Ca, const T* bsrc, int Cb, T* out, float* part, int HW, int G,
-                                                   int S) {
+                                                   int S, long lda, long ldb, long ldo) {
   __shared__ float sm_red[4][2 * GN_GB];
   const int C = Ca + Cb;
   const int s = blockIdx.x, g0 = blockIdx.y * GN_GB, b = blockIdx.z, cpg = div_small(C, rcp_fast(G));
@@ -480,7 +485,7 @@
   const int r0 = div_small(HW * s, inv_S), r1 = div_small(HW * (s + 1), inv_S);
   const int rr = div_small((int)threadIdx.x, inv_nch), ch = threadIdx.x - rr * nch;
   auto load8 = [&](size_t m, int n) {
-    return n < Ca ? *reinterpret_cast<const uint4*>(a + m * Ca + n) : *reinterpret_cast<const uint4*>(bsrc + m * Cb + (n - Ca));
+    return n < Ca ? *reinterpret_cast<const uint4*>(a + m * lda + n) : *reinterpret_cast<const uint4*>(bsrc + m * ldb + (n - Ca));
   };
   float ga[GN_GB], gq[GN_GB], pg[GN_GB];
 #pragma unroll
@@ -489,7 +494,7 @@
     if (g0 + gl < G) {
       const int n = (g0 + gl) * cpg;
       const size_t m = (size_t)b * HW + r0;
-      pg[gl] = to_f32<T>(n < Ca ? a[m * Ca + n] : bsrc[m * Cb + (n - Ca)]);
+      pg[gl] = to_f32<T>(n < Ca ? a[m * lda + n] : bsrc[m * ldb + (n - Ca)]);
     }
   }
   if (rr < RP && g0 * cpg + ch * 8 < C) {
@@ -507,7 +512,7 @@
     for (int r = r0 + rr; r < r1; r += RP) {
       const size_t m = (size_t)b * HW + r;
       const uint4 raw = load8(m, n);
-      *reinterpret_cast<uint4*>(out + m * C + n) = raw;
+      *reinterpret_cast<uint4*>(out + m * ldo + n) = raw;
       const T* v = reinterpret_cast<const T*>(&raw);
 #pragma unroll
       for (int i = 0; i < 8; ++i) { const float d = to_f32<T>(v[i]) - pv[i]; av[i] += d; qv[i] += d * d; }
@@ -541,14 +546,17 @@
 }
 
 void launch_concat_gn(int dtype, const void* a, int Ca, const void* b, int Cb, void* out, float* gn_part, int B, int HW,
-                      int G, hipStream_t st) {
+                      int G, hipStream_t st, long lda, long ldb, long ldo) {
   DH_ABLATE(8);
+  if (lda <= 0) lda = Ca;
+  if (ldb <= 0) ldb = Cb;
+  if (ldo <= 0) ldo = Ca + Cb;
   const int S = gn_slices(HW, B);
   dim3 grid(S, cdiv(G, GN_GB), B);
   if (dtype == DH_DTYPE_F16)
-    hipLaunchKernelGGL((k_concat_gn<f16>), grid, dim3(256), 0, st, (const f16*)a, Ca, (const f16*)b, Cb, (f16*)out, gn_part, HW, G, S);
+    hipLaunchKernelGGL((k_concat_gn<f16>), grid, dim3(256), 0, st, (const f16*)a, Ca, (const f16*)b, Cb, (f16*)out, gn_part, HW, G, S, lda, ldb, ldo);
   else
-    hipLaunchKernelGGL((k_concat_gn<bf16>), grid, dim3(256), 0, st, (const bf16*)a, Ca, (const bf16*)b, Cb, (bf16*)out, gn_part, HW, G, S);
+    hipLaunchKernelGGL((k_concat_gn<bf16>), grid, dim3(256), 0, st, (const bf16*)a, Ca, (const bf16*)b, Cb, (bf16*)out, gn_part, HW, G, S, lda, ldb, ldo);
 }
 
 constexpr int LN_MAXCH = 8;
```

Measured after the change: 36.62 steps/s, median of 6. No clear change (+0.9%).
